# yh-jun/SNR-Aligned_diffSE

Hardware: AMD Instinct MI355X
Metric: utterances/sec (4 s @16 kHz, N=30 PC steps) at 1/2/4/8 MI355X; PESQ delta vs ref (higher is better)
Workload: dtype fp16; 1 GPU; C2: B=32 4 s/16 kHz clips per GPU, N=30 PC steps (reverse_diffusion + ald, 60 NFE/utt), OUVE SDE, NCSN++ nf=128, fp16; global_batch=32, per_gpu_batch=32, seq_len=512, parallelism=dp1 (utterance sharding)

## Files before the change

include/snrse.h:

```cpp
#ifndef SNRSE_H_
#define SNRSE_H_

#include <stddef.h>
#include <stdint.h>

#ifdef __cplusplus
extern "C" {
#endif

typedef struct ihipStream_t* hipStream_t;

enum { SNRSE_F32 = 0, SNRSE_BF16 = 1, SNRSE_F16 = 2, SNRSE_F64 = 3, SNRSE_F32X3 = 4 };

int snrse_abi_version(void);
const char* snrse_build_id(void);
const char* snrse_error_string(int code);
int snrse_device_name(char* buf, int len);

typedef struct snrse_ctx snrse_ctx;
snrse_ctx* snrse_ctx_create(void);
void snrse_ctx_destroy(snrse_ctx* ctx);
int snrse_ctx_set_workspace(snrse_ctx* ctx, void* ptr, size_t bytes);
int snrse_ctx_set_option(snrse_ctx* ctx, const char* name, int value);
int snrse_ctx_get_option(const snrse_ctx* ctx, const char* name, int* value);
int snrse_ctx_probe_begin(snrse_ctx* ctx, int capacity);
int snrse_ctx_probe_read(snrse_ctx* ctx, float* ms, int* kernel, int max, int* n);

int snrse_upfirdn2d(const void* in, void* out, const float* kernel, int major, int in_h, int in_w,
                    int minor, int kh, int kw, int up_x, int up_y, int down_x, int down_y,
                    int pad_x0, int pad_x1, int pad_y0, int pad_y1, int dtype, hipStream_t stream);

int snrse_conv2d(snrse_ctx* ctx, const void* src0, int C0, const void* src1, int C1, int B, int H, int W, int ksize,
                 const void* wgt, const void* sc_src, int Csc, const void* sc_src1, int Csc1,
                 const void* sc_wgt, const float* bias, const float* temb, int temb_stride,
                 const void* res, int res_ld, float out_scale, const float* comb_src,
                 const float* comb_w, const float* comb_b, void* out, int Cout, int out_ld,
                 double* stats, const float* gn_scale, const float* gn_shift, int gn_act, int dtype,
                 int out_f32, hipStream_t stream);

#define SNRSE_STAT_SLOTS 16

int snrse_gn_stats(snrse_ctx* ctx, const void* src0, int C0, const void* src1, int C1, int B, int HW, double* sums,
                   double* sums1, int dtype, hipStream_t stream);

int snrse_gn_scale_shift(const double* sums0, int C0, const double* sums1, int C1, int B, int HW,
                         const float* gamma, const float* beta, int groups, float eps, float* scale,
                         float* shift, hipStream_t stream);

int snrse_gn_apply(const void* src0, int C0, const void* src1, int C1, int B, int H, int W,
                   const double* sums, const double* sums1, const float* gamma, const float* beta,
                   int groups, float eps, int act, int mode, void* out, int dtype, hipStream_t stream);

int snrse_gn_resample(snrse_ctx* ctx, const void* src, int C, int B, int H, int W, const float* scale, const float* shift,
                      int act, int mode, void* out_act, void* out_raw, int dtype, hipStream_t stream);

int snrse_gn_act(const void* src0, int C0, const void* src1, int C1, int B, int HW, const float* scale,
                 const float* shift, int act, void* out, int dtype, hipStream_t stream);

int snrse_set_workspace(void* ptr, size_t bytes);

int snrse_set_option(const char* name, int value);

int snrse_get_option(const char* name, int* value);

int snrse_attention(const void* qkv, void* out, int B, int L, int C, int dtype, hipStream_t stream);

int snrse_temb_mlp(const float* t, const float* Wg, const float* W1, const float* b1, const float* W2,
                   const float* b2, float* temb, int B, int nf, hipStream_t stream);
int snrse_temb_gfp_dense(const float* t, const float* Wg, const float* W1, const float* b1, float* out, int B, int nf,
                         hipStream_t stream);
int snrse_temb_dense(const float* temb, const float* W, const float* bias, float* out, int B, int R, int D,
                     hipStream_t stream);

int snrse_input_conv(snrse_ctx* ctx, const void* x, const void* y, int B, int H, int W, const void* wgt, const float* bias,
                     void* out, float* pyr, double* stats, int dtype, hipStream_t stream);

int snrse_input_conv_x3(snrse_ctx* ctx, const void* x, const void* y, int B, int H, int W, const void* wgt,
                        const float* bias, float* out, float* pyr, double* stats, hipStream_t stream);

int snrse_input_pack(const void* x, const void* y, int B, int H, int W, void* col, float* pyr, int dtype,
                     hipStream_t stream);

int snrse_score_update(const void* pyr, int pyr_f32, const float* out_w, const float* out_b,
                       const float* t, int score_mode, int B, int HW, const void* x, const void* y,
                       const void* noise, uint64_t seed, uint64_t offset, const float* coef,
                       void* x_out, void* xmean_out, void* score_out, hipStream_t stream);

int snrse_sde_update(const void* x, const void* y, const void* score, const void* noise, uint64_t seed,
                     uint64_t offset, const float* coef, int B, int HW, void* x_out, void* xmean_out,
                     hipStream_t stream);

int snrse_axpby_noise(const void* x, const void* y, const void* noise, uint64_t seed, uint64_t offset,
                      const float* coef, int B, int HW, void* out, hipStream_t stream);

int snrse_score_update_rs(const void* pyr, int pyr_f32, const float* out_w, const float* out_b,
                          const float* t, int score_mode, int B, int HW, const void* x, const void* y,
                          const void* noise, const uint64_t* row_seed, uint64_t draw, const float* coef,
                          void* x_out, void* xmean_out, void* score_out, hipStream_t stream);
int snrse_sde_update_rs(const void* x, const void* y, const void* score, const void* noise,
                        const uint64_t* row_seed, uint64_t draw, const float* coef, int B, int HW, void* x_out,
                        void* xmean_out, hipStream_t stream);
int snrse_axpby_noise_rs(const void* x, const void* y, const void* noise, const uint64_t* row_seed,
                         uint64_t draw, const float* coef, int B, int HW, void* out, hipStream_t stream);

int snrse_energy_ratios(const float* s_hat, const float* s, const float* n, int B, int L, double* out,
                        hipStream_t stream);

int snrse_absmax(const float* sig, int B, int L, float* out, hipStream_t stream);

int snrse_energy_ratios_ragged(const float* s_hat, const float* s, const float* n, const int* lengths, int B,
                               int Lstride, double* out, hipStream_t stream);
int snrse_absmax_ragged(const float* sig, const int* lengths, int B, int Lstride, float* out, hipStream_t stream);
int snrse_stft_ragged(const float* sig, const int* lengths, int B, int Lstride, const float* in_div,
                      float in_scale, int Tpad, int mode, void* out, hipStream_t stream);

int snrse_resample_poly(const float* x, const int* lengths, int B, long long stride_in, int up, int down, int half,
                        const float* taps, float* y, long long stride_out, hipStream_t stream);
int snrse_resample_poly_block(void);

int snrse_window_gather(const float* src, const int* lengths, int R, long long stride, const int* table, int nwin,
                        int W, float* out, hipStream_t stream);
int snrse_window_merge(const float* win, int nwin, int W, const int* starts, const unsigned char* silent,
                       const int* first, const int* lengths, int R, const float* fade, int V, float* out,
                       long long stride_out, hipStream_t stream);

int snrse_estoi(const float* x, const float* y, const int* lengths, int B, long long stride, void* work,
                size_t work_bytes, double* out, int* info, hipStream_t stream);
size_t snrse_estoi_workspace(int B, long long stride);
int snrse_estoi_block(void);

int snrse_range_stats(const void* src, int B, long long per, int dtype, float* peak, int* nonfinite,
                      int accumulate, hipStream_t stream);


int snrse_rk45_combine(const double* y, const double* h, const void* const* k, const double* c, int ns, int kdtype,
                       int B, long long n, double* out, float* out32, hipStream_t stream);

int snrse_rk45_rownorm(const void* const* v, const double* c, int ns, int vdtype, const double* m, const double* a,
                       const double* b2, double rtol, double atol, int cplx, int B, long long n, double* partial,
                       double* out, hipStream_t stream);
int snrse_rk45_rownorm_blocks(int B, long long n);

int snrse_rk45_accept(const int* mask, void* y, const void* y_new, long long ywords, void* f, const void* f_new,
                      long long fwords, int B, hipStream_t stream);

int snrse_stft(const float* sig, int B, int L, const float* in_div, float in_scale, int Tpad, int mode,
               void* out, hipStream_t stream);

int snrse_istft(const void* spec, int B, int T, int L, int mode, const float* out_scale, float* frames,
                float* out, hipStream_t stream);

int snrse_spec_transform(const void* in, void* out, long long n, int dir, hipStream_t stream);

int snrse_snrnet(const void* spec, int B, int T, const float* w5, const float* b5, const float* w3,
                 const float* b3, const float* wt1, const float* wt2, const float* wt3, const float* wt4,
                 const float* bt1, const float* bt2, const float* bt3, const float* bt4, const float* wih,
                 const float* bsum, const float* whh, const float* fcw, const float* fcb, float* ws,
                 float* out, hipStream_t stream);
size_t snrse_snrnet_workspace(int B, int T);


int snrse_snr_perturb(const void* x, const void* y, const float* gt, int B, long long per, void* out,
                      hipStream_t stream);
int snrse_snrnet_train_fwd(const void* spec, int B, int T, const float* w5, const float* b5, const float* w3,
                           const float* b3, const float* wt1, const float* wt2, const float* wt3, const float* wt4,
                           const float* bt1, const float* bt2, const float* bt3, const float* bt4, const float* wih,
                           const float* bsum, const float* whh, const float* fcw, const float* fcb, void* tws,
                           float* out, hipStream_t stream);
size_t snrse_snrnet_train_workspace(int B, int T);
int snrse_snrnet_backward(const void* spec, int B, int T, const float* est, const float* dest, const float* w3,
                          const float* wt1, const float* wt2, const float* wt3, const float* wt4, const float* wih,
                          const float* whh, const float* fcw, void* tws, float* dw5, float* db5, float* dw3,
                          float* db3, float* dwt1, float* dwt2, float* dwt3, float* dwt4, float* dbt1, float* dbt2,
                          float* dbt3, float* dbt4, float* dwih, float* dbsum, float* dwhh, float* dfcw, float* dfcb,
                          hipStream_t stream);


int snrse_conv_wgrad(const float* dy, int Cout, const float* x0, int C0, const float* x1, int C1, int B, int H,
                     int W, int ksize, float* dw, hipStream_t stream);
int snrse_conv_wgrad_x3(const float* dy, int Cout, const float* x0, int C0, const float* x1, int C1, int B, int H,
                        int W, int ksize, float* dw, hipStream_t stream);
int snrse_chan_sum(const float* x, int B, int HW, int C, float* out_bc, float* out_c, float scale,
                   hipStream_t stream);
int snrse_gn_moments(const double* st0, int C0, const double* st1, int C1, int B, int HW, int groups, float eps,
                     float* mean, float* rstd, hipStream_t stream);
int snrse_gn_backward(const float* x0, int C0, const float* x1, int C1, const float* dy, int B, int HW,
                      int groups, const float* gamma, const float* beta, const float* mean, const float* rstd,
                      int act, float* R, float* dx0, float* dx1, float* dgamma, float* dbeta, hipStream_t stream);
int snrse_bgemm(const float* A, long long sAb, long long sAm, long long sAk, const float* Bm, long long sBb,
                long long sBk, long long sBn, float* C, long long sCb, long long sCm, long long sCn, const float* bias,
                int batch, int M, int N, int K, float alpha, float beta, hipStream_t stream);
int snrse_softmax_rows(const float* S, float* P, long long rows, int L, float scale, hipStream_t stream);
int snrse_softmax_bwd_rows(const float* P, const float* dP, float* dS, long long rows, int L, float scale,
                           hipStream_t stream);
int snrse_silu(const float* x, float* y, long long n, hipStream_t stream);
int snrse_silu_bwd(const float* x, const float* dy, float* dx, long long n, int accumulate, hipStream_t stream);
int snrse_axpby(const float* x, float* y, long long n, float a, float b, hipStream_t stream);
int snrse_scale_rows(const float* x, const float* s, float* y, int B, long long per, int recip, hipStream_t stream);
int snrse_gfp(const float* t, const float* Wg, int B, int nf, float* out, hipStream_t stream);
int snrse_ct_perturb(const void* x, const void* y, const void* z, const float* wmix, const float* nscale, int B,
                     int HW, int transform, void* mu, void* xt, hipStream_t stream);
int snrse_ct_loss(const void* dnn1, const void* dnn0, const void* x1, const void* x0, const float* coef, int B,
                  int HW, int sqrt_loss, double* loss_b, void* g1, void* g0, hipStream_t stream);
int snrse_adam_ema(const void* tensors, const int* chunk_tensor, const long long* chunk_start, int nchunks,
                   float lr, float beta1, float beta2, float eps, float bias_corr1, float bias_corr2_sqrt,
                   float ema_decay, hipStream_t stream);
int snrse_grad_sumsq(const void* tensors, const int* chunk_tensor, const long long* chunk_start, int nchunks,
                     double* partial, hipStream_t stream);
int snrse_grad_clip_coef(const double* partial, int npartials, float max_norm, float accum_scale, float* out,
                         hipStream_t stream);
int snrse_adam_ema_scaled(const void* tensors, const int* chunk_tensor, const long long* chunk_start, int nchunks,
                          float lr, float beta1, float beta2, float eps, float bias_corr1, float bias_corr2_sqrt,
                          float ema_decay, const float* gscale, hipStream_t stream);
int snrse_grad_pack(const void* tensors, const int* chunk_tensor, const long long* chunk_start, int nchunks,
                    const long long* flat_off, float scale, float* flat, hipStream_t stream);


int snrse_active_window_sums(const float* c, const float* n, const int* lengths, int B, long long stride, int W,
                             double* wsums, double* partials, float* nmax, hipStream_t stream);
int snrse_active_windows_per_block(void);
int snrse_active_finalize(const double* wsums, const double* partials, const float* nmax, const int* lengths, int B,
                          long long stride, int W, const double* snr_db, double* out, hipStream_t stream);
int snrse_snr_mix(const float* c, const float* n, const int* lengths, int B, long long stride, const double* gain,
                  int gain_stride, float* n_out, float* y_out, float* ymax, hipStream_t stream);
int snrse_scale_to_pcm16(const float* c, const float* n1, const float* y, const int* lengths, int B, long long stride,
                         const float* ymax, float* c_f, float* n_f, float* y_f, short* c_q, short* n_q, short* y_q,
                         double* scale, hipStream_t stream);

#ifdef __cplusplus
}
#endif
#endif
```

snr-aligned_diffse_amd/csrc/abi.cpp:

```cpp
#include <hip/hip_runtime.h>

#include <new>

#include "common.h"

extern "C" int snrse_abi_version(void) { return 2; }

#ifndef SNRSE_BUILD_ID
#define SNRSE_BUILD_ID "unknown"
#endif
extern "C" const char* snrse_build_id(void) { return SNRSE_BUILD_ID; }

extern "C" const char* snrse_error_string(int code) { return hipGetErrorString((hipError_t)code); }

extern "C" int snrse_device_name(char* buf, int len) {
  int dev = 0;
  hipError_t e = hipGetDevice(&dev);
  if (e != hipSuccess) return (int)e;
  hipDeviceProp_t prop;
  e = hipGetDeviceProperties(&prop, dev);
  if (e != hipSuccess) return (int)e;
  int i = 0;
  for (const char* s = prop.gcnArchName; *s && i < len - 1; ++s) buf[i++] = *s;
  if (len > 0) buf[i] = 0;
  return 0;
}

namespace {
snrse_ctx g_default_ctx;

bool name_is(const char* a, const char* b) {
  int i = 0;
  while (a[i] && a[i] == b[i]) ++i;
  return a[i] == 0 && b[i] == 0;
}

int* option_field(snrse_ctx& c, const char* name) {
  if (name_is(name, "conv_variant")) return &c.conv_variant;
  if (name_is(name, "splitk")) return &c.splitk;
  if (name_is(name, "splitk_target")) return &c.splitk_target;
  if (name_is(name, "epi_nt")) return &c.epi_nt;
  if (name_is(name, "epi_nt_mb")) return &c.epi_nt_mb;
  if (name_is(name, "h5_specialise")) return &c.h5_specialise;
  if (name_is(name, "h5_tw")) return &c.h5_tw;
  if (name_is(name, "stats_zeroed")) return &c.stats_zeroed;
  if (name_is(name, "resample_variant")) return &c.resample_variant;
  if (name_is(name, "resample_nt")) return &c.resample_nt;
  if (name_is(name, "resample_down_rows")) return &c.resample_down_rows;
  if (name_is(name, "x3_tile")) return &c.x3_tile;
  if (name_is(name, "x3_spread")) return &c.x3_spread;
  if (name_is(name, "ic_lds")) return &c.ic_lds;
  if (name_is(name, "x3_nt")) return &c.x3_nt;
  if (name_is(name, "x3_tw")) return &c.x3_tw;
  if (name_is(name, "head_small")) return &c.head_small;
  if (name_is(name, "head_part")) return &c.head_part;
  if (name_is(name, "gn_slice")) return &c.gn_slice;
  return nullptr;
}

int set_option(snrse_ctx& c, const char* name, int value) {
  if (!name) return SNRSE_EINVAL;
  int* f = option_field(c, name);
  if (!f) return SNRSE_EINVAL;
  if (name_is(name, "splitk_target") || name_is(name, "epi_nt_mb")) value = value > 0 ? value : 256;
  if (name_is(name, "stats_zeroed")) value = value ? 1 : 0;
  *f = value;
  return 0;
}

int get_option(const snrse_ctx& c, const char* name, int* value) {
  if (!name || !value) return SNRSE_EINVAL;
  if (const int* f = option_field(const_cast<snrse_ctx&>(c), name)) { *value = *f; return 0; }
  if (name_is(name, "halo_kernel")) { *value = 5; return 0; }
  if (name_is(name, "last_kernel")) { *value = c.last_kernel; return 0; }
  if (name_is(name, "last_ksplit")) { *value = c.last_ksplit; return 0; }
  if (name_is(name, "last_epi_nt")) { *value = c.last_epi_nt; return 0; }
  if (name_is(name, "last_chunks")) { *value = c.last_chunks; return 0; }
  if (name_is(name, "last_tw")) { *value = c.last_tw; return 0; }
  return SNRSE_EINVAL;
}

int set_workspace(snrse_ctx& c, void* ptr, size_t bytes) {
  if (!ptr && bytes) return SNRSE_EINVAL;
  c.ws = (float*)ptr;
  c.ws_bytes = ptr ? bytes : 0;
  return 0;
}
}

__attribute__((visibility("hidden"))) snrse_ctx* snrse_ctx_resolve(snrse_ctx* c) { return c ? c : &g_default_ctx; }

namespace {
void probe_free(snrse_ctx& c) {
  for (int i = 0; i < 2 * c.probe_cap; ++i) (void)hipEventDestroy(c.probe_ev[i]);
  delete[] c.probe_ev;
  delete[] c.probe_kernel;
  c.probe_ev = nullptr;
  c.probe_kernel = nullptr;
  c.probe_cap = c.probe_n = 0;
}
}

__attribute__((visibility("hidden"))) int snrse_ctx_probe_mark(snrse_ctx& c, hipStream_t s, bool end) {
  if (c.probe_n >= c.probe_cap) return 0;
  if (end) {
    c.probe_kernel[c.probe_n] = c.last_kernel;
    return (int)hipEventRecord(c.probe_ev[2 * c.probe_n++ + 1], s);
  }
  return (int)hipEventRecord(c.probe_ev[2 * c.probe_n], s);
}

extern "C" int snrse_ctx_probe_begin(snrse_ctx* ctx, int capacity) {
  snrse_ctx& c = *snrse_ctx_resolve(ctx);
  probe_free(c);
  if (capacity <= 0) return 0;
  c.probe_ev = new (std::nothrow) hipEvent_t[2 * (size_t)capacity];
  c.probe_kernel = new (std::nothrow) int[capacity];
  if (!c.probe_ev || !c.probe_kernel) {
    delete[] c.probe_ev;
    delete[] c.probe_kernel;
    c.probe_ev = nullptr;
    c.probe_kernel = nullptr;
    return (int)hipErrorOutOfMemory;
  }
  for (int i = 0; i < 2 * capacity; ++i) {
    const hipError_t e = hipEventCreateWithFlags(&c.probe_ev[i], hipEventDisableSystemFence);
    if (e != hipSuccess) {
      c.probe_cap = i / 2;
      for (int j = 2 * c.probe_cap; j < i; ++j) (void)hipEventDestroy(c.probe_ev[j]);
      probe_free(c);
      return (int)e;
    }
  }
  c.probe_cap = capacity;
  c.probe_n = 0;
  return 0;
}

extern "C" int snrse_ctx_probe_read(snrse_ctx* ctx, float* ms, int* kernel, int max, int* n) {
  snrse_ctx& c = *snrse_ctx_resolve(ctx);
  if (!n) return SNRSE_EINVAL;
  const int m = c.probe_n < max ? c.probe_n : max;
  for (int i = 0; i < m; ++i) {
    hipError_t e = hipEventSynchronize(c.probe_ev[2 * i + 1]);
    if (e != hipSuccess) return (int)e;
    if (ms) {
      e = hipEventElapsedTime(&ms[i], c.probe_ev[2 * i], c.probe_ev[2 * i + 1]);
      if (e != hipSuccess) return (int)e;
    }
    if (kernel) kernel[i] = c.probe_kernel[i];
  }
  *n = m;
  return 0;
}

extern "C" snrse_ctx* snrse_ctx_create(void) {
  snrse_ctx* c = new (std::nothrow) snrse_ctx(g_default_ctx);
  if (!c) return nullptr;
  c->ws = nullptr;
  c->ws_bytes = 0;
  c->last_kernel = 0;
  c->last_ksplit = 1;
  c->last_epi_nt = 0;
  c->last_chunks = 1;
  c->last_tw = 0;
  c->probe_ev = nullptr;
  c->probe_kernel = nullptr;
  c->probe_cap = c->probe_n = 0;
  return c;
}

extern "C" void snrse_ctx_destroy(snrse_ctx* ctx) {
  if (ctx) probe_free(*ctx);
  delete ctx;
}

extern "C" int snrse_ctx_set_workspace(snrse_ctx* ctx, void* ptr, size_t bytes) {
  return set_workspace(*snrse_ctx_resolve(ctx), ptr, bytes);
}
extern "C" int snrse_ctx_set_option(snrse_ctx* ctx, const char* name, int value) {
  return set_option(*snrse_ctx_resolve(ctx), name, value);
}
extern "C" int snrse_ctx_get_option(const snrse_ctx* ctx, const char* name, int* value) {
  return get_option(*snrse_ctx_resolve(const_cast<snrse_ctx*>(ctx)), name, value);
}

extern "C" int snrse_set_workspace(void* ptr, size_t bytes) { return set_workspace(g_default_ctx, ptr, bytes); }
extern "C" int snrse_set_option(const char* name, int value) { return set_option(g_default_ctx, name, value); }
extern "C" int snrse_get_option(const char* name, int* value) { return get_option(g_default_ctx, name, value); }
```

snr-aligned_diffse_amd/csrc/common.h:

```cpp
#pragma once
#include <hip/hip_runtime.h>
#include <stdint.h>

#define SNRSE_DEV __device__ __forceinline__

typedef uint16_t bf16_t;

typedef __attribute__((ext_vector_type(8))) __bf16 bf16x8_mfma;
typedef __attribute__((ext_vector_type(4))) float f32x4;
typedef __attribute__((ext_vector_type(4))) unsigned int u32x4;

SNRSE_DEV float bf2f(bf16_t v) { return __uint_as_float(((uint32_t)v) << 16); }

SNRSE_DEV bf16_t f2bf(float f) {
  uint32_t u = __float_as_uint(f);
  if ((u & 0x7f800000u) == 0x7f800000u && (u & 0x007fffffu)) return (bf16_t)((u >> 16) | 0x40);
  u += 0x7fffu + ((u >> 16) & 1u);
  return (bf16_t)(u >> 16);
}

SNRSE_DEV uint32_t pack_bf16x2(float lo, float hi) {
  typedef __attribute__((ext_vector_type(2))) __bf16 bf16x2_t;
  const bf16x2_t v = {(__bf16)lo, (__bf16)hi};
  return __builtin_bit_cast(uint32_t, v);
}

struct f16_t {
  uint16_t bits;
};
typedef __attribute__((ext_vector_type(8))) _Float16 f16x8_mfma;
typedef __attribute__((ext_vector_type(2))) _Float16 f16x2_t;

template <typename T> struct H16;
template <> struct H16<bf16_t> {
  SNRSE_DEV static float lo(uint32_t v) { return __uint_as_float(v << 16); }
  SNRSE_DEV static float hi(uint32_t v) { return __uint_as_float(v & 0xffff0000u); }
  SNRSE_DEV static uint32_t pack(float a, float b) { return pack_bf16x2(a, b); }
  SNRSE_DEV static f32x4 mfma(const u32x4& a, const u32x4& b, f32x4 acc) {
    return __builtin_amdgcn_mfma_f32_16x16x32_bf16(__builtin_bit_cast(bf16x8_mfma, a),
                                                   __builtin_bit_cast(bf16x8_mfma, b), acc, 0, 0, 0);
  }
};
template <> struct H16<f16_t> {
  SNRSE_DEV static float lo(uint32_t v) { return (float)__builtin_bit_cast(f16x2_t, v)[0]; }
  SNRSE_DEV static float hi(uint32_t v) { return (float)__builtin_bit_cast(f16x2_t, v)[1]; }
  SNRSE_DEV static uint32_t pack(float a, float b) {
    const f16x2_t v = {(_Float16)a, (_Float16)b};
    return __builtin_bit_cast(uint32_t, v);
  }
  SNRSE_DEV static f32x4 mfma(const u32x4& a, const u32x4& b, f32x4 acc) {
    return __builtin_amdgcn_mfma_f32_16x16x32_f16(__builtin_bit_cast(f16x8_mfma, a),
                                                  __builtin_bit_cast(f16x8_mfma, b), acc, 0, 0, 0);
  }
};
template <typename T>
SNRSE_DEV void unpack8(const u32x4& r, float* v) {
#pragma unroll
  for (int i = 0; i < 4; ++i) {
    v[2 * i] = H16<T>::lo(r[i]);
    v[2 * i + 1] = H16<T>::hi(r[i]);
  }
}
template <typename T>
SNRSE_DEV u32x4 pack8(const float* v) {
  u32x4 r;
#pragma unroll
  for (int i = 0; i < 4; ++i) r[i] = H16<T>::pack(v[2 * i], v[2 * i + 1]);
  return r;
}

template <typename T> struct Elem;
template <> struct Elem<float> {
  static constexpr int kBytes = 4;
  SNRSE_DEV static float to_f(float v) { return v; }
  SNRSE_DEV static float from_f(float v) { return v; }
};
template <> struct Elem<bf16_t> {
  static constexpr int kBytes = 2;
  SNRSE_DEV static float to_f(bf16_t v) { return bf2f(v); }
  SNRSE_DEV static bf16_t from_f(float v) { return f2bf(v); }
};
template <> struct Elem<f16_t> {
  static constexpr int kBytes = 2;
  SNRSE_DEV static float to_f(f16_t v) { return (float)__builtin_bit_cast(_Float16, v.bits); }
  SNRSE_DEV static f16_t from_f(float v) { return f16_t{__builtin_bit_cast(uint16_t, (_Float16)v)}; }
};

SNRSE_DEV float silu(float x) { return x * __builtin_amdgcn_rcpf(1.0f + __expf(-x)); }
constexpr float kNegLog2e = -1.44269504088896341f;
constexpr float kNegInvLn2 = -1.44269504088896341f;
SNRSE_DEV float silu_z(float z) {
  return z * __builtin_amdgcn_rcpf(fmaf(__builtin_amdgcn_exp2f(z), kNegInvLn2, kNegInvLn2));
}

SNRSE_DEV float silu_exact(float x) { return x / (1.0f + expf(-x)); }

SNRSE_DEV float wave_sum(float v) {
#pragma unroll
  for (int o = 32; o > 0; o >>= 1) v += __shfl_xor(v, o, 64);
  return v;
}
SNRSE_DEV float wave_max(float v) {
#pragma unroll
  for (int o = 32; o > 0; o >>= 1) v = fmaxf(v, __shfl_xor(v, o, 64));
  return v;
}
template <int N>
SNRSE_DEV float bfly_sum(float (&p)[N], int lane) {
  static_assert(N >= 1 && N <= 64 && (N & (N - 1)) == 0, "N: power of two <= 64");
  int lb = 0;
#pragma unroll
  for (int n = N; n > 1; n >>= 1, ++lb) {
    const bool hi = (lane >> lb) & 1;
#pragma unroll
    for (int i = 0; i < n / 2; ++i) {
      const float keep = hi ? p[2 * i + 1] : p[2 * i];
      const float send = hi ? p[2 * i] : p[2 * i + 1];
      p[i] = keep + __shfl_xor(send, 1 << lb, 64);
    }
  }
  float v = p[0];
#pragma unroll
  for (int b = lb; b < 6; ++b) v += __shfl_xor(v, 1 << b, 64);
  return v;
}

SNRSE_DEV int xcd_block_id(int bid, int nblocks) {
  const int q8 = nblocks >> 3, r8 = nblocks & 7, xcd = bid & 7, pos = bid >> 3;
  return (xcd < r8 ? xcd * (q8 + 1) : r8 * (q8 + 1) + (xcd - r8) * q8) + pos;
}

SNRSE_DEV float dot4(const f32x4& a, const f32x4& b) {
  return fmaf(a[0], b[0], fmaf(a[1], b[1], fmaf(a[2], b[2], a[3] * b[3])));
}

SNRSE_DEV double wave_sum_d(double v) {
#pragma unroll
  for (int o = 32; o > 0; o >>= 1) v += __shfl_xor(v, o, 64);
  return v;
}

enum { SNRSE_F32 = 0, SNRSE_BF16 = 1, SNRSE_F16 = 2, SNRSE_F64 = 3, SNRSE_F32X3 = 4 };
inline bool snrse_is16(int dtype) { return dtype == SNRSE_BF16 || dtype == SNRSE_F16; }

#define SNRSE_STAT_SLOTS 16

struct snrse_ctx {
  int conv_variant = 0;
  int splitk = 1;
  int splitk_target = 256;
  int epi_nt = 2;
  int epi_nt_mb = 256;
  int h5_specialise = 1;
  int h5_tw = 0;
  int stats_zeroed = 0;
  int resample_variant = 0;
  int resample_nt = 0;
  int resample_down_rows = 4;
  int x3_tile = 0;
  int x3_tw = 0;
  int x3_nt = 1;
  int x3_spread = 2;
  int head_small = 1;
  int head_part = 1;
  int gn_slice = 1;
  int ic_lds = 3;
  float* ws = nullptr;
  size_t ws_bytes = 0;
  int last_kernel = 0, last_ksplit = 1, last_epi_nt = 0, last_chunks = 1, last_tw = 0;
  hipEvent_t* probe_ev = nullptr;
  int* probe_kernel = nullptr;
  int probe_cap = 0, probe_n = 0;
};
int snrse_ctx_probe_mark(snrse_ctx& c, hipStream_t s, bool end);
snrse_ctx* snrse_ctx_resolve(snrse_ctx* c);
SNRSE_DEV size_t stat_idx(int b, int slot, int c, int C) {
  return (((size_t)b * SNRSE_STAT_SLOTS + slot) * C + c) * 2;
}
SNRSE_DEV void stat_fold(const double* st, int b, int c, int C, double& s, double& ss) {
#pragma unroll 4
  for (int k = 0; k < SNRSE_STAT_SLOTS; ++k) {
    const double* q = st + stat_idx(b, k, c, C);
    s += q[0];
    ss += q[1];
  }
}

#define SNRSE_RET(expr)                              \
  do {                                               \
    hipError_t _e = (expr);                          \
    if (_e != hipSuccess) return (int)_e;            \
  } while (0)
#define SNRSE_LAUNCH_CHECK() SNRSE_RET(hipGetLastError())
#define SNRSE_EINVAL ((int)hipErrorInvalidValue)
```

snr-aligned_diffse_amd/csrc/conv.hip:

```cpp
#include "conv_common.h"

#include <algorithm>
#include <type_traits>

using namespace snrse_conv;

namespace {

template <int NWM, int BN>
SNRSE_DEV void block_stats_flush(const ConvParams& p, const float* red, int blk_b, int blk_n0) {
  asm volatile("s_waitcnt lgkmcnt(0)" ::: "memory");
  __builtin_amdgcn_s_barrier();
  const int slot = blockIdx.x & (SNRSE_STAT_SLOTS - 1);
  for (int t = threadIdx.x; t < 2 * BN; t += blockDim.x) {
    float a = 0.f;
#pragma unroll
    for (int w = 0; w < NWM; ++w) a += red[w * 2 * BN + t];
    if (blk_n0 + (t >> 1) < p.Cout)
      unsafeAtomicAdd(&p.stats[stat_idx(blk_b, slot, blk_n0 + (t >> 1), p.Cout) + (t & 1)], (double)a);
  }
}

template <typename TO, int NWM, int BN, bool DEFER = false, int LA = 8>
SNRSE_DEV void epilogue_lds(const ConvParams& p, const f32x4 (&acc)[4][4], int mb, int nb, int lane, float* stage,
// ... 894 lines not shown
        wait_vm(infl ? HOPS : 0);
        __builtin_amdgcn_s_barrier();
        char* const nxt = ring + (SLOT2 - so);
        if constexpr (k < 8) {
          wtap(c0 + (2 * k + 2) / 9, (2 * k + 2) % 9, nxt);
          wtap(c0 + (2 * k + 3) / 9, (2 * k + 3) % 9, nxt + TAPB);
        } else {
          if (more) {
            wtap(c0 + 2, 0, nxt);
            wtap(c0 + 2, 1, nxt + TAPB);
          } else if (cbs > 0) {
            wtap(cbm, 4, nxt);
          }
        }
        infl = false;
        if constexpr (k == 0) {
          halo_load(c1);
          infl = true;
        }
        if constexpr (k == 4) {
          if (pf1) {
            halo_load(c1 + 1);
            infl = true;
          }
        }
        const char* const sl_ = ring + so;
        auto piece_after = [&](int d, int t) {
          const int c = c0 + d;
          if (t < 4 || t > 7) return;
          if (d == 1 && !pf1) return;
          char* const nb_ = smem + ((c + 1) & 1) * HBYTES;
          const bool tr = c + 1 < cbm;
          if (t == 4) { halo_piece(nb_, 0, tr); halo_piece(nb_, 1, tr); }
          if (t == 5) { halo_piece(nb_, 2, tr); halo_piece(nb_, 3, tr); }
          if (t == 6) halo_piece(nb_, 4, tr);
          if (t == 7) halo_piece(nb_, 5, tr);
        };
        tap_mfma(smem + ((c0 + da) & 1) * HBYTES, sl_, ta);
        piece_after(da, ta);
        __builtin_amdgcn_sched_barrier(0);
        tap_mfma(smem + ((c0 + db) & 1) * HBYTES, sl_ + TAPB, tb);
        piece_after(db, tb);
        __builtin_amdgcn_sched_barrier(0);
        so = SLOT2 - so;
      });
    }
    for (int c = cbm; c < ncb; ++c) {
      asm volatile("s_waitcnt vmcnt(0) lgkmcnt(0)" ::: "memory");
      __builtin_amdgcn_s_barrier();
      if (c + 1 < ncb) wtap(c + 1, 4, ring + (SLOT2 - so));
      if (c + 1 < ncb) halo_load(c + 1);
      tap_mfma(smem + (c & 1) * HBYTES, ring + so, 4);
      if (c + 1 < ncb) {
        asm volatile("s_waitcnt vmcnt(0)" ::: "memory");
        char* const nb_ = smem + ((c + 1) & 1) * HBYTES;
#pragma unroll
        for (int j = 0; j < HJ; ++j) halo_piece(nb_, j, false);
      }
      so = SLOT2 - so;
    }
  } else if constexpr (SPR == 1) {
    int q = 0;
    for (int c = 0; c < cbm; ++c) {
      const bool tr = c + 1 < cbm;
      char* const nb_ = smem + ((c + 1) & 1) * HBYTES;
      const char* const hb = smem + (c & 1) * HBYTES;
#pragma unroll
      for (int tp = 0; tp < 9; ++tp, ++q) {
        if (tp == 1) asm volatile("s_waitcnt vmcnt(%0)" ::"n"(2 + HOPS) : "memory");
        else asm volatile("s_waitcnt vmcnt(2)" ::: "memory");
        asm volatile("s_waitcnt lgkmcnt(0)" ::: "memory");
        __builtin_amdgcn_s_barrier();
        wload(q + 2);
        if (tp == 0) halo_load(c + 1 < ncb ? c + 1 : c);
        tap_mfma(hb, ring + (q % 3) * TAPB, tp);
        if (tp >= 2 && tp - 2 < HJ) halo_piece(nb_, tp - 2, tr);
      }
    }
    for (int c = cbm; c < ncb; ++c, ++q) {
      const int qa = q - 2, qb = q - 1;
      const bool fa = qa >= 0 && (qa >= 9 * cbm || qa % 9 == 0), fb = qb >= 0 && (qb >= 9 * cbm || qb % 9 == 0);
      x3h_vm_wait(2 + HOPS * (int)fa + HOPS * (int)fb);
      asm volatile("s_waitcnt lgkmcnt(0)" ::: "memory");
      __builtin_amdgcn_s_barrier();
      wload(q + 2);
      halo_load(c + 1 < ncb ? c + 1 : c);
      tap_mfma(smem + (c & 1) * HBYTES, ring + (q % 3) * TAPB, 4);
      asm volatile("s_waitcnt vmcnt(0)" ::: "memory");
      char* const nb_ = smem + ((c + 1) & 1) * HBYTES;
#pragma unroll
      for (int j = 0; j < HJ; ++j) halo_piece(nb_, j, false);
    }
  } else
  for (int q = 0; q < nq; ++q) {
    const int c = phase_chunk(q), tp = phase_tap(q);
    x3h_vm_wait(HOPS * (int)first_with_next(q - 2) + 2 * (int)(q + 1 < nq) + HOPS * (int)first_with_next(q - 1));
    asm volatile("s_waitcnt lgkmcnt(0)" ::: "memory");
    __builtin_amdgcn_s_barrier();
    if (q + 2 < nq) wload(q + 2);
    const bool pre = first_with_next(q);
    if (pre) halo_load(c + 1);
    const char* hb = smem + (c & 1) * HBYTES;
    const char* sb = ring + (q % 3) * TAPB;
    const int dy = tp / 3 - 1, dx = tp - (tp / 3) * 3 - 1;
    const int hbase = (wr * RW + dy + 1) * HC + dx + 1 + lrow;
    u32x4 ah[4], al[4], bh[4], bl[4];
#pragma unroll
    for (int i = 0; i < 4; ++i) {
      const int hr = hbase + (16 * i / TW) * HC + (16 * i) % TW;
      ah[i] = *(const u32x4*)(hb + swz(hr, lg));
      al[i] = *(const u32x4*)(hb + swz(hr, 4 + lg));
    }
#pragma unroll
    for (int j = 0; j < 4; ++j) {
      bh[j] = *(const u32x4*)(sb + swz(wc * 64 + j * 16 + lrow, lg));
      bl[j] = *(const u32x4*)(sb + swz(wc * 64 + j * 16 + lrow, 4 + lg));
    }
#pragma unroll
    for (int i = 0; i < 4; ++i)
#pragma unroll
      for (int j = 0; j < 4; ++j) {
        acc[i][j] = mfma_chunk<bf16_t>(ah[i], bh[j], acc[i][j]);
        acc[i][j] = mfma_chunk<bf16_t>(ah[i], bl[j], acc[i][j]);
        acc[i][j] = mfma_chunk<bf16_t>(al[i], bh[j], acc[i][j]);
      }
    const int q0 = q < 9 * cbm ? q - tp : q;
    const bool last_of_chunk = c < cbm ? tp == 8 : true;
    const bool store_now = c + 1 < ncb && (c < cbm ? tp == 1 : true);
    if (store_now) {
      x3h_vm_wait(q == q0 ? 0 : 2 * (int)(q0 + 3 < nq));
      halo_store(c + 1);
    }
    (void)last_of_chunk;
  }
  asm volatile("s_waitcnt vmcnt(0) lgkmcnt(0)" ::: "memory");
  __builtin_amdgcn_s_barrier();
  const int mb = (bb * p.H + h0 + wr * RW) * p.W + w0;
  if constexpr (TW == 64)
    epilogue_lds<float, 4, 128>(p, acc, mb, n0 + wc * 64, lane, (float*)(smem + wid * (64 * 68 * 4)),
                                (float*)(smem + 8 * (64 * 68 * 4)), wr, bb, n0, min(TW, p.W - w0));
  else
    epilogue_img<float, 4, 128, false, EF, TW>(p, acc, mb, n0 + wc * 64, lane, (float*)(smem + wid * (64 * 68 * 4)),
                                                 (float*)(smem + 8 * (64 * 68 * 4)), wr, bb, n0, p.W - TW);
}

template <int BM, int BN, typename T, typename TO>
__global__ __launch_bounds__(512) void conv_glds_kernel(ConvParams p) {
  constexpr int WM = BM / 64, WN = BN / 64;
  static_assert(WM * WN == 8, "8 waves");
  constexpr int FM = 4, FN = 4, TM = 64, TN = 64;
  constexpr int STAGES = 3;
  constexpr int A_BYTES = BM * 128, B_BYTES = BN * 128, STAGE = A_BYTES + B_BYTES;
  constexpr int AJ = BM / 64, BJ = BN / 64;
  constexpr int KT = 64;
  extern __shared__ __attribute__((aligned(16))) char smem[];

  const int tid = threadIdx.x, lane = tid & 63;
  const int wid = __builtin_amdgcn_readfirstlane(tid >> 6);
  const int wm = wid / WN, wn = wid % WN;
  const int wg = xcd_block_id(blockIdx.x, gridDim.x);
  const int ks = wg % p.ksplit, tl = wg / p.ksplit;
  const int m0 = (tl / p.ntn) * BM;
  const int n0 = (tl % p.ntn) * BN;

  const int HW = p.H * p.W;
  const int Cin = p.C0 + p.C1;
  const int cblocks = Cin / KT;
  const int nk0 = p.ksize * p.ksize * cblocks;
  const int Csc_all = p.Csc + p.Csc1;
  const int nk = nk0 + (p.sc_src ? Csc_all / KT : 0);
  const int K1 = p.ksize * p.ksize * Cin;
  const int half = p.ksize >> 1;
  const int slot = lane & 7;

  int a_pix[AJ], a_h[AJ], a_w[AJ], a_ch[AJ];
  bool a_ok[AJ];
#pragma unroll
  for (int j = 0; j < AJ; ++j) {
    const int row = (wid * AJ + j) * 8 + (lane >> 3);
    const int m = m0 + row;
    a_ok[j] = m < p.M;
    const int mm = a_ok[j] ? m : 0;
    const int b = mm / HW, rem = mm - b * HW;
    a_h[j] = rem / p.W;
    a_w[j] = rem - a_h[j] * p.W;
    a_pix[j] = mm;
    a_ch[j] = slot ^ (row & 7);
  }

#define SNRSE_ISSUE(KT_, STAGE_)                                                                      \
  do {                                                                                              \
    const int kt_ = (KT_);                                                                          \
    char* sa_ = smem + (STAGE_) * STAGE;                                                            \
    char* sb_ = sa_ + A_BYTES;                                                                      \
    int cs_, cc_, dy_, dx_, wld_, koff_;                                                            \
    const void* abase_;                                                                             \
    long long abytes_;                                                                              \
    const void* wbase_;                                                                             \
    long long wbytes_;                                                                              \
    if (kt_ < nk0) {                                                                                \
      const int tap_ = kt_ / cblocks;                                                               \
      const int c_ = (kt_ - tap_ * cblocks) * KT;                                                   \
      dy_ = tap_ / p.ksize - half;                                                                  \
      dx_ = tap_ - (tap_ / p.ksize) * p.ksize - half;                                               \
      const bool u1_ = c_ >= p.C0;                                                                  \
      abase_ = u1_ ? p.src1 : p.src0;                                                               \
      abytes_ = u1_ ? p.bytes1 : p.bytes0;                                                          \
      cs_ = u1_ ? p.C1 : p.C0;                                                                      \
      cc_ = u1_ ? c_ - p.C0 : c_;                                                                   \
      wbase_ = p.wgt;                                                                               \
      wbytes_ = p.wbytes;                                                                           \
      wld_ = K1;                                                                                    \
      koff_ = tap_ * Cin + c_;                                                                      \
    } else {                                                                                        \
      const int c_ = (kt_ - nk0) * KT;                                                              \
      const bool u1_ = c_ >= p.Csc;                                                                 \
      abase_ = u1_ ? p.sc_src1 : p.sc_src;                                                          \
      abytes_ = u1_ ? p.sc_bytes1 : p.sc_bytes0;                                                    \
      cs_ = u1_ ? p.Csc1 : p.Csc;                                                                   \
      cc_ = u1_ ? c_ - p.Csc : c_;                                                                  \
      dy_ = 0;                                                                                      \
      dx_ = 0;                                                                                      \
      wbase_ = p.sc_wgt;                                                                            \
      wbytes_ = p.sc_wbytes;                                                                        \
      wld_ = Csc_all;                                                                               \
      koff_ = c_;                                                                                   \
    }                                                                                               \
    const __amdgpu_buffer_rsrc_t ra_ = make_rsrc(abase_, abytes_);                                  \
    const __amdgpu_buffer_rsrc_t rb_ = make_rsrc(wbase_, wbytes_);                                  \
    const int shift_ = dy_ * p.W + dx_;                                                             \
    _Pragma("unroll") for (int j = 0; j < AJ; ++j) {                                                \
      const int hh_ = a_h[j] + dy_, ww_ = a_w[j] + dx_;                                             \
      const bool ok_ = a_ok[j] && hh_ >= 0 && hh_ < p.H && ww_ >= 0 && ww_ < p.W;                   \
      const unsigned voff_ =                                                                        \
          ok_ ? (unsigned)(((a_pix[j] + shift_) * cs_ + cc_ + a_ch[j] * 8) * 2) : 0x80000000u;      \
      __builtin_amdgcn_raw_ptr_buffer_load_lds(                                                     \
          ra_, (__attribute__((address_space(3))) void*)(sa_ + (wid * AJ + j) * 1024), 16, voff_, 0, 0, 0); \
    }                                                                                               \
    _Pragma("unroll") for (int j = 0; j < BJ; ++j) {                                                \
      const int row_ = (wid * BJ + j) * 8 + (lane >> 3);                                            \
      const int chk_ = slot ^ (row_ & 7);                                                           \
      const unsigned voff_ = (unsigned)(((n0 + row_) * wld_ + koff_ + chk_ * 8) * 2);               \
      __builtin_amdgcn_raw_ptr_buffer_load_lds(                                                     \
          rb_, (__attribute__((address_space(3))) void*)(sb_ + (wid * BJ + j) * 1024), 16, voff_, 0, 0, 0); \
    }                                                                                               \
  } while (0)

  f32x4 acc[FM][FN];
#pragma unroll
  for (int i = 0; i < FM; ++i)
#pragma unroll
    for (int j = 0; j < FN; ++j) acc[i][j] = f32x4{0.f, 0.f, 0.f, 0.f};

  const int kb = (int)((long long)ks * nk / p.ksplit), ke = (int)((long long)(ks + 1) * nk / p.ksplit);
  SNRSE_ISSUE(kb, 0);
  if (ke - kb > 1) SNRSE_ISSUE(kb + 1, 1);
  const int lrow = lane & 15, lg = lane >> 4;
  int stage = 0;
  for (int kt = kb; kt < ke; ++kt) {
    if (kt + 1 < ke)
      asm volatile("s_waitcnt vmcnt(%0)" ::"n"(AJ + BJ) : "memory");
    else
      asm volatile("s_waitcnt vmcnt(0)" ::: "memory");
    __builtin_amdgcn_s_barrier();
    if (kt + 2 < ke) SNRSE_ISSUE(kt + 2, stage == 0 ? 2 : stage - 1);
    const char* sa = smem + stage * STAGE;
    const char* sb = sa + A_BYTES;
#pragma unroll
    for (int s = 0; s < 2; ++s) {
      u32x4 af[FM], bfr[FN];
#pragma unroll
      for (int i = 0; i < FM; ++i) af[i] = *(const u32x4*)(sa + swz(wm * TM + i * 16 + lrow, 4 * s + lg));
#pragma unroll
      for (int j = 0; j < FN; ++j) bfr[j] = *(const u32x4*)(sb + swz(wn * TN + j * 16 + lrow, 4 * s + lg));
#pragma unroll
      for (int i = 0; i < FM; ++i)
#pragma unroll
        for (int j = 0; j < FN; ++j) acc[i][j] = mfma_chunk<T>(af[i], bfr[j], acc[i][j]);
    }
    stage = stage == STAGES - 1 ? 0 : stage + 1;
  }
#undef SNRSE_ISSUE
  if (p.ksplit > 1) {
    float* const wsp = p.ws + (size_t)ks * p.M * p.Cout;
#pragma unroll
    for (int i = 0; i < FM; ++i)
#pragma unroll
      for (int e = 0; e < 4; ++e) {
        const int m = m0 + wm * TM + i * 16 + lg * 4 + e;
        if (m < p.M) {
#pragma unroll
          for (int j = 0; j < FN; ++j) wsp[(size_t)m * p.Cout + n0 + wn * TN + j * 16 + lrow] = acc[i][j][e];
        }
      }
    return;
  }
  asm volatile("s_waitcnt vmcnt(0) lgkmcnt(0)" ::: "memory");
  __builtin_amdgcn_s_barrier();
  const int b_lo = m0 / HW, b_hi = (min(m0 + BM, p.M) - 1) / HW;
  epilogue_lds<TO, WM, BN, false, sizeof(TO) == 2 ? 8 : 1>(p, acc, m0 + wm * TM, n0 + wn * TN, lane, (float*)(smem + wid * (64 * 68 * 4)),
                           (float*)(smem + 8 * (64 * 68 * 4)), wm, b_lo == b_hi ? b_lo : -1, n0);
}

template <typename TO>
__global__ __launch_bounds__(256) void conv_splitk_finalize(ConvParams p, int ppb) {
  __shared__ float red[16 * 256];
  const int HW = p.H * p.W;
  const int nbi = (HW + ppb - 1) / ppb;
  const int b = blockIdx.x / nbi;
  const int px0 = (blockIdx.x - b * nbi) * ppb, px1 = min(HW, px0 + ppb);
  const int cl = (threadIdx.x & 15) * 8, r0 = threadIdx.x >> 4;
  const int n = blockIdx.y * 128 + cl;
  float add[8], cw[8][4], cb[8], s1[8], s2[8];
#pragma unroll
  for (int k = 0; k < 8; ++k) {
    add[k] = (p.bias ? p.bias[n + k] : 0.f) + (p.temb ? p.temb[(size_t)b * p.temb_stride + n + k] : 0.f);
    s1[k] = 0.f;
    s2[k] = 0.f;
    cb[k] = 0.f;
    cw[k][0] = cw[k][1] = cw[k][2] = cw[k][3] = 0.f;
    if (p.comb_src) {
      cw[k][0] = p.comb_w[(n + k) * 4 + 0];
      cw[k][1] = p.comb_w[(n + k) * 4 + 1];
      cw[k][2] = p.comb_w[(n + k) * 4 + 2];
      cw[k][3] = p.comb_w[(n + k) * 4 + 3];
      cb[k] = p.comb_b[n + k];
    }
  }
  const size_t plane = (size_t)p.M * p.Cout;
  for (int px = px0 + r0; px < px1; px += 16) {
    const size_t m = (size_t)b * HW + px;
    const float* w = p.ws + m * p.Cout + n;
    f32x4 a0 = *(const f32x4*)w, a1 = *(const f32x4*)(w + 4);
    int s = 1;
    for (; s + 4 <= p.ksplit; s += 4) {
      f32x4 q[4][2];
#pragma unroll
      for (int u = 0; u < 4; ++u) {
        q[u][0] = *(const f32x4*)(w + (s + u) * plane);
        q[u][1] = *(const f32x4*)(w + (s + u) * plane + 4);
      }
#pragma unroll
      for (int u = 0; u < 4; ++u) {
        a0 += q[u][0];
        a1 += q[u][1];
      }
    }
    for (; s < p.ksplit; ++s) {
      a0 += *(const f32x4*)(w + s * plane);
      a1 += *(const f32x4*)(w + s * plane + 4);
    }
    float v[8];
#pragma unroll
    for (int k = 0; k < 4; ++k) {
      v[k] = a0[k] + add[k];
      v[4 + k] = a1[k] + add[4 + k];
    }
    if (p.res) {
      if constexpr (sizeof(TO) == 2) {
        epi_residual<TO>(*(const u32x4*)((const TO*)p.res + m * p.res_ld + n), v);
      } else {
        const float* rp = (const float*)p.res + m * p.res_ld + n;
#pragma unroll
        for (int k = 0; k < 8; ++k) v[k] += rp[k];
      }
    }
#pragma unroll
    for (int k = 0; k < 8; ++k) v[k] *= p.out_scale;
    if (p.comb_src) {
      const f32x4 q = *(const f32x4*)(p.comb_src + m * 4);
#pragma unroll
      for (int k = 0; k < 8; ++k) v[k] += q[0] * cw[k][0] + q[1] * cw[k][1] + q[2] * cw[k][2] + q[3] * cw[k][3] + cb[k];
    }
    if constexpr (sizeof(TO) == 2) {
      *(u32x4*)((TO*)p.out + m * p.out_ld + n) = epi_pack<TO>(v);
    } else {
      float* op = (float*)p.out + m * p.out_ld + n;
#pragma unroll
      for (int k = 0; k < 8; ++k) op[k] = v[k];
    }
#pragma unroll
    for (int k = 0; k < 8; ++k) {
      s1[k] += v[k];
      s2[k] = fmaf(v[k], v[k], s2[k]);
    }
  }
  if (p.stats) {
#pragma unroll
    for (int k = 0; k < 8; ++k) {
      red[r0 * 256 + (cl + k) * 2] = s1[k];
      red[r0 * 256 + (cl + k) * 2 + 1] = s2[k];
    }
    __syncthreads();
    const int t = threadIdx.x;
    float a = 0.f;
#pragma unroll
    for (int r = 0; r < 16; ++r) a += red[r * 256 + t];
    unsafeAtomicAdd(&p.stats[stat_idx(b, blockIdx.x & (SNRSE_STAT_SLOTS - 1), blockIdx.y * 128 + (t >> 1), p.Cout) +
                             (t & 1)],
                    (double)a);
  }
}


template <typename T, typename TO, int GNM, int EF, int TW, bool SCD>
__global__ __launch_bounds__(256, 2) void conv_halo5_kernel(ConvParams p) {
  constexpr int TH = 256 / TW, HC = TW + 2;
  constexpr int RW = TH / 4;
  constexpr int HROWS = (TH + 2) * HC;
  constexpr int HJ = (HROWS + 63) / 64;
  constexpr int HALO_BYTES = HROWS * 64;
  constexpr int TAPB = 128 * 64;
  constexpr int SLOT = 3 * TAPB;
  constexpr int KT = 32;
  static_assert(64 * HJ >= HROWS, "halo rows");
  extern __shared__ __attribute__((aligned(16))) char smem[];
  char* const halo = smem;
  char* const ring = smem + HALO_BYTES;
  float* const gnl = (float*)(smem + HALO_BYTES + 2 * SLOT + 1024);
  constexpr bool REGEPI = sizeof(TO) == 2;
  constexpr int MAIN_BYTES = HALO_BYTES + 2 * SLOT + 1280;
  constexpr int STAGE_BYTES = 4 * (64 * 68 * 4);

  const int tid = threadIdx.x, lane = tid & 63;
  const int wid = __builtin_amdgcn_readfirstlane(tid >> 6);
#ifdef SNRSE_STAMPS
  constexpr int kStampOff = REGEPI ? MAIN_BYTES + 4096
                                   : (MAIN_BYTES > STAGE_BYTES + 4096 ? MAIN_BYTES : STAGE_BYTES + 4096);
  unsigned long long* const lst = (unsigned long long*)(smem + kStampOff) + wid * 32;
#endif
  SNRSE_STAMP(0);
  const int wg = xcd_block_id(blockIdx.x, gridDim.x);
  const int n0 = (wg % p.ntn) * 128;
  int tile = wg / p.ntn;
  const int ntw = p.W / TW, nth = p.H / TH;
  const int w0 = (tile % ntw) * TW;
  tile /= ntw;
  const int h0 = (tile % nth) * TH;
  const int bb = tile / nth;

  const int Cin = p.C0 + p.C1;
  const int cbm = Cin / KT;
  const int Csc_all = p.Csc + p.Csc1;
  const int cbs = p.sc_src ? Csc_all / KT : 0;
  const int nq = 3 * cbm + cbs;
  const int K1 = 9 * Cin;
  const int hcol = tid & 3;

  const int rl = lane >> 2, swz8 = ((lane & 3) ^ ((rl >> 1) & 3)) * 8;
  const __amdgpu_buffer_rsrc_t wrsrc = make_rsrc(p.wgt, p.wbytes);
  const int wr0 = REGEPI ? 8 * rl + wid : wid * 16 + rl;
  constexpr int WODD = REGEPI ? 4 : 64;
  const unsigned wlane = (unsigned)(((n0 + wr0) * K1 + swz8) * 2);
  const unsigned wrow64 = (unsigned)(WODD * K1 * 2), wtap = (unsigned)(Cin * 2);
  using lds_ptr = __attribute__((address_space(3))) void*;
  auto dma_w = [&](auto k_, unsigned vl, unsigned soff, char* dst) {
    constexpr int k = decltype(k_)::value;
    __builtin_amdgcn_raw_ptr_buffer_load_lds(wrsrc, (lds_ptr)(dst + (k >> 1) * TAPB + (wid + 4 * (k & 1)) * 1024), 16,
                                             vl, soff + (k & 1) * wrow64 + (k >> 1) * wtap, 0, 0);
  };
  auto woff = [&](int c, int g) { return (unsigned)((3 * g * Cin + c * KT) * 2); };

  u32x4 hv[HJ];
  f32x4 gnv;
  auto gn_load = [&](int c) {
    if constexpr (GNM > 0) {
      if (tid < 16)
        gnv = *(const f32x4*)((tid < 8 ? p.gn_scale : p.gn_shift) + (size_t)bb * Cin + c * KT + (tid & 7) * 4);
    }
  };

  static_for<6>([&](auto k) { dma_w(k, wlane, 0u, ring); });
  gn_load(0);
  __builtin_amdgcn_sched_barrier(0);

  int hpix[HJ];
  bool hok[HJ];
#pragma unroll
  for (int j = 0; j < HJ; ++j) {
    const int hr = (tid >> 2) + 64 * j;
    const int hy = hr / HC, hx = hr - (hr / HC) * HC;
    const int ih = h0 + hy - 1, iw = w0 + hx - 1;
    hok[j] = hr < HROWS && ih >= 0 && ih < p.H && iw >= 0 && iw < p.W;
    hpix[j] = (bb * p.H + ih) * p.W + iw;
  }

#define SNRSE_HALO5_LOADS(BASE_, BYTES_, CS_, CC_)                                                     \
  do {                                                                                              \
    const __amdgpu_buffer_rsrc_t r_ = make_rsrc((BASE_), (BYTES_));                                 \
    const int cs_ = (CS_), cc_ = (CC_) + hcol * 8;                                                  \
    _Pragma("unroll") for (int j = 0; j < HJ; ++j) {                                                \
      const int voff_ = hok[j] ? (hpix[j] * cs_ + cc_) * 2 : (int)0x80000000;                       \
      hv[j] = __builtin_amdgcn_raw_buffer_load_b128(r_, voff_, 0, 0);                               \
    }                                                                                               \
  } while (0)
  auto halo_load = [&](int c) {
    const int ch = c * KT;
    const bool s1 = ch >= p.C0;
    SNRSE_HALO5_LOADS(s1 ? p.src1 : p.src0, s1 ? p.bytes1 : p.bytes0, s1 ? p.C1 : p.C0, s1 ? ch - p.C0 : ch);
  };
#undef SNRSE_HALO5_LOADS
  auto gn_publish = [&]() {
    if constexpr (GNM > 0) {
      if (tid < 16) {
        f32x4 g = gnv;
        if constexpr (GNM == 2) g *= kNegLog2e;
        *(f32x4*)(gnl + tid * 4) = g;
      }
    }
  };
  auto halo_store = [&](int c) {
    const bool tr = GNM > 0;
    float gsc[8], gsh[8];
    if constexpr (GNM > 0) {
      if (tr) {
        const f32x4 s0 = *(const f32x4*)(gnl + hcol * 8), s1 = *(const f32x4*)(gnl + hcol * 8 + 4);
        const f32x4 t0 = *(const f32x4*)(gnl + 32 + hcol * 8), t1 = *(const f32x4*)(gnl + 32 + hcol * 8 + 4);
#pragma unroll
        for (int i = 0; i < 4; ++i) { gsc[i] = s0[i]; gsc[4 + i] = s1[i]; gsh[i] = t0[i]; gsh[4 + i] = t1[i]; }
      }
    }
#pragma unroll
    for (int j = 0; j < HJ; ++j) {
      const int hr = (tid >> 2) + 64 * j;
      if (j == HJ - 1 && hr >= HROWS) break;
      u32x4 v = hv[j];
      if constexpr (GNM > 0) {
        if (tr) v = gn_xform8<T, GNM>(v, gsc, gsh, hok[j]);
      }
      *(u32x4*)(halo + swz64(hr, hcol)) = v;
    }
  };
  f32x4 acc[2][4][4];
#pragma unroll
  for (int h = 0; h < 2; ++h)
#pragma unroll
    for (int i = 0; i < 4; ++i)
#pragma unroll
      for (int j = 0; j < 4; ++j) acc[h][i][j] = f32x4{0.f, 0.f, 0.f, 0.f};
  const int lrow = lane & 15, lg = lane >> 4;
  auto vm_after_dma = [&]() { __builtin_amdgcn_s_waitcnt(0x0f76); };


  if constexpr (SCD) {
    const int kq = cbs / cbm, kr = cbs - kq * cbm;
    int krem = 0;
    auto nsc_next = [&]() {
      krem += kr;
      const bool wrap = krem >= cbm;
      if (wrap) krem -= cbm;
      return kq + (wrap ? 1 : 0);
    };
    auto kind_of = [](int s, int k, int& su) -> int {
      su = 0;
      if (k >= 3) {
        if (s == 0 || s == 2 || s == 4) return s >> 1;
        su = s <= 3 ? s >> 1 : s - 3;
        return 3;
      }
      if (s < 2) return s;
      if (k == 0) return 2;
      if (k == 1) {
        if (s == 2) return 2;
        return 3;
      }
      if (s == 3) return 2;
      su = s == 2 ? 0 : 1;
      return 3;
    };
    auto m2_pos = [](int k) { return k >= 3 ? 4 : k == 2 ? 3 : 2; };
    const __amdgpu_buffer_rsrc_t scrsrc = make_rsrc(p.sc_wgt, p.sc_wbytes);
    const __amdgpu_buffer_rsrc_t xrsrc0 = make_rsrc(p.sc_src, p.sc_bytes0), xrsrc1 = make_rsrc(p.sc_src1, p.sc_bytes1);
    const unsigned sclane = (unsigned)(((n0 + wr0) * Csc_all + swz8) * 2);
    const unsigned scrow64 = (unsigned)(WODD * Csc_all * 2);
    const int trow = wid * 16 + rl;
    const int xpix = (bb * p.H + h0 + trow / TW) * p.W + w0 + trow % TW;
    halo_load(0);
    if constexpr (GNM > 0) {
      gn_publish();
      __syncthreads();
    }
    halo_store(0);
    const bool w0g = GNM > 0 && wid == 0;
    bool halo_inflight = false;
    int c = 0, pos = 0, k = nsc_next(), ub = 0;
    int su, kind = kind_of(0, k, su);
    for (int q = 0; q < nq; ++q) {
      int c2 = c, pos2 = pos + 1, k2 = k, ub2 = ub;
      if (pos2 == 3 + k) { c2 = c + 1; pos2 = 0; ub2 = ub + k; k2 = c2 < cbm ? nsc_next() : 0; }
      int su2;
      const int kind2 = kind_of(pos2, k2, su2);
      if (halo_inflight) {
        if (w0g) asm volatile("s_waitcnt vmcnt(%0) lgkmcnt(0)" ::"n"(HJ + 1) : "memory");
        else asm volatile("s_waitcnt vmcnt(%0) lgkmcnt(0)" ::"n"(HJ) : "memory");
      } else {
        asm volatile("s_waitcnt vmcnt(0) lgkmcnt(0)" ::: "memory");
      }
      __builtin_amdgcn_s_barrier();
      char* const nx = ring + ((q + 1) & 1) * SLOT;
      __amdgpu_buffer_rsrc_t Rc, Rn;
      unsigned Vc, Vn, Sc, Sn, Oc, On, DPn;
      int DDn;
      char* Dc = nx + wid * 1024;
      char* Dn = Dc + TAPB;
      if (kind2 < 3) {
        const bool fin = q + 1 >= nq;
        Rc = Rn = wrsrc;
        Vc = Vn = fin ? wlane | 0x80000000u : wlane;
        Sc = fin ? 0u : woff(c2, kind2);
        Sn = Sc + wtap; DPn = wtap; DDn = TAPB;
        Oc = On = wrow64;
      } else {
        const int kb = (ub2 + su2) * KT;
        const bool one = kb >= p.Csc;
        const int cs = one ? p.Csc1 : p.Csc, cb = one ? kb - p.Csc : kb;
        const unsigned xstep = (unsigned)((64 / TW) * p.W * cs * 2);
        Rc = scrsrc; Vc = sclane; Sc = (unsigned)(kb * 2); Oc = scrow64;
        Rn = one ? xrsrc1 : xrsrc0;
        Vn = (unsigned)((xpix * cs + swz8) * 2);
        Sn = (unsigned)(cb * 2); On = xstep; DPn = 2 * xstep; DDn = 8192;
      }
      auto dma_pair = [&]() {
        __builtin_amdgcn_raw_ptr_buffer_load_lds(Rc, (lds_ptr)Dc, 16, Vc, Sc, 0, 0);
        __builtin_amdgcn_raw_ptr_buffer_load_lds(Rc, (lds_ptr)(Dc + 4096), 16, Vc, Sc + Oc, 0, 0);
        Rc = Rn; Vc = Vn; Sc = Sn; Oc = On; Dc = Dn;
        Sn += DPn; Dn += DDn;
      };
      const char* sl = ring + (q & 1) * SLOT;
      const bool mainph = kind < 3;
      const char* abuf = mainph ? halo : sl + TAPB;
      const int ntap = mainph ? 3 : 1, rs = mainph ? HC : TW;
      const int arow0 = mainph ? (wid * RW + kind) * HC + lrow : wid * RW * TW + lrow;
      auto tap_body = [&](int jt, auto gap_) {
        constexpr bool gap = decltype(gap_)::value;
        const int arow = arow0 + jt;
        const char* sb = sl + jt * TAPB;
        u32x4 af[4], bfr[8];
#pragma unroll
        for (int i = 0; i < 4; ++i) af[i] = *(const u32x4*)(abuf + swz64(arow + (16 * i / TW) * rs + (16 * i) % TW, lg));
#pragma unroll
        for (int j = 0; j < 8; ++j) bfr[j] = *(const u32x4*)(sb + swz64(j * 16 + lrow, lg));
        static_for<32>([&](auto m_) {
          constexpr int m = decltype(m_)::value, h = m >> 4, i = (m >> 2) & 3, j = m & 3;
          acc[h][i][j] = mfma_chunk<T>(af[i], bfr[h * 4 + j], acc[h][i][j]);
          if constexpr (gap && (m & 7) == 7 && m < 24) dma_pair();
        });
        if constexpr (gap) {
#pragma unroll
          for (int u = 0; u < 3; ++u) {
            __builtin_amdgcn_sched_group_barrier(0x008, 8, 0);
            __builtin_amdgcn_sched_group_barrier(0x020, 2, 0);
          }
          __builtin_amdgcn_sched_group_barrier(0x008, 8, 0);
        }
      };
      tap_body(0, std::true_type{});
#pragma nounroll
      for (int jt = 1; jt < ntap; ++jt) tap_body(jt, std::false_type{});
      if (kind == 0 && c + 1 < cbm) {
        vm_after_dma();
        halo_load(c + 1);
        gn_load(c + 1);
        halo_inflight = true;
      } else {
        halo_inflight = false;
      }
      if (c + 1 < cbm) {
        if (kind == 2) {
          gn_publish();
          if (k == 0) {
            asm volatile("s_waitcnt lgkmcnt(0)" ::: "memory");
            __builtin_amdgcn_s_barrier();
            vm_after_dma();
            halo_store(c + 1);
          }
        } else if (kind == 3 && pos == m2_pos(k) + 1) {
          vm_after_dma();
          halo_store(c + 1);
        }
      }
      c = c2; pos = pos2; k = k2; ub = ub2; kind = kind2; su = su2;
    }
  } else {
  halo_load(0);
  if constexpr (GNM > 0) {
    gn_publish();
    __syncthreads();
  }
  halo_store(0);
  SNRSE_STAMP(1);
  bool halo_inflight = false;
  const bool w0g = GNM > 0 && wid == 0;
  int c = 0, g = 0;
  unsigned soff = woff(0, 1);
  const unsigned soff_g = 3 * wtap, soff_c = (unsigned)(2 * KT) - 6 * wtap;
  for (int q = 0; q < nq; ++q) {
    const bool first = g == 0, last = g == 2;
    if (halo_inflight) {
      if (w0g) asm volatile("s_waitcnt vmcnt(%0) lgkmcnt(0)" ::"n"(HJ + 1) : "memory");
      else asm volatile("s_waitcnt vmcnt(%0) lgkmcnt(0)" ::"n"(HJ) : "memory");
    } else {
      asm volatile("s_waitcnt vmcnt(0) lgkmcnt(0)" ::: "memory");
    }
    __builtin_amdgcn_s_barrier();
    SNRSE_STAMP(2 + 2 * (q & 15));
    const bool fin = q + 1 >= nq;
    const unsigned vl = fin ? wlane | 0x80000000u : wlane, so = fin ? 0u : soff;
    char* const nx = ring + ((q + 1) & 1) * SLOT;
    const char* sl = ring + (q & 1) * SLOT;
    const int hrow = (wid * RW + g) * HC + lrow;
    static_for<3>([&](auto jt_) {
      constexpr int jt = decltype(jt_)::value;
      const int hbase = hrow + jt;
      const char* sb = sl + jt * TAPB;
      u32x4 af[4], bfr[8];
#pragma unroll
      for (int i = 0; i < 4; ++i) af[i] = *(const u32x4*)(halo + swz64(hbase + (16 * i / TW) * HC + (16 * i) % TW, lg));
#pragma unroll
      for (int j = 0; j < 8; ++j) bfr[j] = *(const u32x4*)(sb + swz64(j * 16 + lrow, lg));
      static_for<32>([&](auto m_) {
        constexpr int m = decltype(m_)::value, h = m >> 4, i = (m >> 2) & 3, j = m & 3;
        acc[h][i][j] = mfma_chunk<T>(af[i], bfr[h * 4 + j], acc[h][i][j]);
        if constexpr (jt < 2 && (m & 7) == 7 && m < 24)
          dma_w(std::integral_constant<int, 3 * jt + (m >> 3)>{}, vl, so, nx);
      });
    });
    static_assert(sizeof(T) == 2, "one MFMA per mfma_chunk");
#pragma unroll
    for (int t = 0; t < 2; ++t) {
#pragma unroll
      for (int u = 0; u < 3; ++u) {
        __builtin_amdgcn_sched_group_barrier(0x008, 8, 0);
        __builtin_amdgcn_sched_group_barrier(0x020, 1, 0);
      }
      __builtin_amdgcn_sched_group_barrier(0x008, 8, 0);
    }
    __builtin_amdgcn_sched_group_barrier(0x008, 32, 0);
    SNRSE_STAMP(3 + 2 * (q & 15));
    if (first && c + 1 < cbm) {
      vm_after_dma();
      halo_load(c + 1);
      gn_load(c + 1);
      halo_inflight = true;
    } else {
      halo_inflight = false;
    }
    if (last && c + 1 < cbm) {
      gn_publish();
      asm volatile("s_waitcnt lgkmcnt(0)" ::: "memory");
      __builtin_amdgcn_s_barrier();
      vm_after_dma();
      halo_store(c + 1);
    }
    soff += g == 1 ? soff_c : soff_g;
    if (last) { g = 0; ++c; }
    else ++g;
  }
  }
  SNRSE_STAMP(28);
#ifdef SNRSE_H5_SKIP_EPI
  if (p.M > 0) {
    asm volatile("s_waitcnt vmcnt(0)" ::: "memory");
    return;
  }
#endif
  const int mrow = (bb * p.H + h0 + wid * RW) * p.W + w0;
  if constexpr (REGEPI) {
    float* const red = (float*)(smem + MAIN_BYTES);
    epilogue_reg<TO, EF, TW>(p, acc, mrow, n0, lane, red + wid * 256, bb, p.W - TW);
    SNRSE_STAMP(26);
    SNRSE_STAMP(27);
    if (EF < 0 ? p.stats != nullptr : (EF & EF_STATS) != 0) block_stats_flush<4, 128>(p, red, bb, n0);
  } else {
    float add0[16 / sizeof(TO)], add1[16 / sizeof(TO)];
    epi_add<TO, EF>(p, n0, lane, bb, add0);
    epi_add<TO, EF>(p, n0 + 64, lane, bb, add1);
    asm volatile("s_waitcnt vmcnt(0) lgkmcnt(0)" ::: "memory");
    __builtin_amdgcn_s_barrier();
    float* const stage = (float*)(smem + wid * (64 * 68 * 4));
    float* const red = (float*)(smem + STAGE_BYTES);
    epilogue_img<TO, 4, 128, true, EF, TW, 2>(p, acc[0], mrow, n0, lane, stage, red, wid, bb, n0, p.W - TW, add0);
    asm volatile("s_waitcnt lgkmcnt(0)" ::: "memory");
    __builtin_amdgcn_wave_barrier();
    SNRSE_STAMP(26);
    epilogue_img<TO, 4, 128, true, EF, TW, 2>(p, acc[1], mrow, n0 + 64, lane, stage, red, wid, bb, n0, p.W - TW, add1);
    SNRSE_STAMP(27);
    if (EF < 0 ? p.stats != nullptr : (EF & EF_STATS) != 0) block_stats_flush<4, 128>(p, red, bb, n0);
  }
#ifdef SNRSE_STAMPS
  {
    unsigned long long st_[29];
    if (lane == 0)
      for (int i = 0; i < 29; ++i) st_[i] = lst[i];
    unsigned long long t_end;
    asm volatile("s_waitcnt vmcnt(0)\n\ts_memtime %0\n\ts_waitcnt lgkmcnt(0)" : "=s"(t_end)::"memory");
    unsigned hw, xcc;
    asm volatile("s_getreg_b32 %0, hwreg(HW_REG_HW_ID)" : "=s"(hw));
    asm volatile("s_getreg_b32 %0, hwreg(HW_REG_XCC_ID)" : "=s"(xcc));
    if (lane == 0 && p.stamps) {
      unsigned long long* g = p.stamps + ((size_t)blockIdx.x * 8 + wid) * 32;
      for (int i = 0; i < 29; ++i) g[i] = st_[i];
      g[29] = t_end;
      g[30] = hw;
      g[31] = xcc;
    }
  }
#endif
}


template <auto K, typename... Args>
int launch_dyn_lds(dim3 grid, dim3 block, size_t lds, hipStream_t s, const Args&... args) {
  static const hipError_t attr = hipFuncSetAttribute((const void*)K, hipFuncAttributeMaxDynamicSharedMemorySize, (int)lds);
  SNRSE_RET(attr);
  hipLaunchKernelGGL(K, grid, block, lds, s, args...);
  return (int)hipGetLastError();
}

template <typename TO>
int launch_splitk_finalize(const ConvParams& p, hipStream_t s) {
  const int HW = p.H * p.W, ppb = 64;
  hipLaunchKernelGGL((conv_splitk_finalize<TO>), dim3(p.B * ((HW + ppb - 1) / ppb), p.Cout / 128), dim3(256), 0, s, p,
                     ppb);
  return (int)hipGetLastError();
}

inline int k_tiles(const ConvParams& p, int KT) {
  return p.ksize * p.ksize * ((p.C0 + p.C1) / KT) + (p.sc_src ? (p.Csc + p.Csc1) / KT : 0);
}

inline int stream_output(const snrse_ctx& cx, long long bytes) {
  return cx.epi_nt == 2 ? bytes > ((long long)cx.epi_nt_mb << 20) : cx.epi_nt;
}

template <typename T, typename TO, int GNM, int EF, int TW, bool SCD>
int launch_halo5_ef(ConvParams p, int grid, hipStream_t s) {
  constexpr size_t main_lds = (256 / TW + 2) * (TW + 2) * 64 + 2 * 3 * 128 * 64 + 1024 + 256;
  constexpr size_t epi_lds = 4 * (64 * 68 * 4) + 4 * 128 * 2 * 4;
  constexpr size_t used_lds = sizeof(TO) == 2 ? main_lds + 4 * 128 * 2 * 4 : (main_lds > epi_lds ? main_lds : epi_lds);
#ifdef SNRSE_STAMPS
  constexpr size_t lds = used_lds + 1024;
#else
  constexpr size_t lds = used_lds;
#endif
  static_assert(lds <= 80 * 1024, "two workgroups per CU");
  return launch_dyn_lds<conv_halo5_kernel<T, TO, GNM, EF, TW, SCD>>(dim3(grid), dim3(256), lds, s, p);
}

template <typename T, typename TO, int GNM, int TW>
int launch_halo5_gn(ConvParams p, hipStream_t s, snrse_ctx& cx) {
  p.ntn = p.Cout / 128;
  p.epi_nt = stream_output(cx, (long long)p.M * p.out_ld * (long long)sizeof(TO));
  cx.last_epi_nt = p.epi_nt;
  const int tiles = p.B * (p.H / (256 / TW)) * (p.W / TW) * p.ntn;
  const int grid = tiles;
  const bool scd = p.sc_src != nullptr;
  if constexpr (sizeof(TO) == 2 && GNM != 1) {
    if (cx.h5_specialise && p.bias) {
#define SNRSE_H5_EF(F) \
  case (F): return launch_halo5_ef<T, TO, GNM, (F), TW, false>(p, grid, s);
#define SNRSE_H5_EFS(F) \
  case (F): return launch_halo5_ef<T, TO, GNM, (F), TW, true>(p, grid, s);
      if (!scd) {
        switch (epi_flags(p)) {
          SNRSE_H5_EF(EF_TEMB | EF_STATS)
          SNRSE_H5_EF(EF_TEMB | EF_STATS | EF_NT)
          SNRSE_H5_EF(EF_RES | EF_STATS)
          SNRSE_H5_EF(EF_RES | EF_STATS | EF_NT)
          SNRSE_H5_EF(EF_STATS)
          SNRSE_H5_EF(EF_STATS | EF_NT)
          SNRSE_H5_EF(EF_TEMB)
          default: break;
        }
      } else {
        switch (epi_flags(p)) {
          SNRSE_H5_EFS(EF_STATS)
          SNRSE_H5_EFS(EF_STATS | EF_NT)
          SNRSE_H5_EFS(EF_COMB | EF_STATS)
          default: break;
        }
      }
#undef SNRSE_H5_EF
#undef SNRSE_H5_EFS
    }
  }
  return scd ? launch_halo5_ef<T, TO, GNM, EF_RT, TW, true>(p, grid, s)
             : launch_halo5_ef<T, TO, GNM, EF_RT, TW, false>(p, grid, s);
}

template <typename T, typename TO, int TW>
int launch_halo5_tw(ConvParams p, hipStream_t s, snrse_ctx& cx) {
  cx.last_tw = TW;
  if (!p.gn_scale) return launch_halo5_gn<T, TO, 0, TW>(p, s, cx);
  if (!p.gn_act) return launch_halo5_gn<T, TO, 1, TW>(p, s, cx);
  return launch_halo5_gn<T, TO, 2, TW>(p, s, cx);
}

inline bool halo_tile32(const ConvParams& p) { return p.H % 8 == 0 && p.W % 32 == 0; }
inline bool halo_tile64(const ConvParams& p) { return p.H % 4 == 0 && p.W % 64 == 0; }

template <typename T, typename TO>
int launch_halo5(ConvParams p, hipStream_t s, snrse_ctx& cx) {
  if (halo_tile32(p) && cx.h5_tw != 64) return launch_halo5_tw<T, TO, 32>(p, s, cx);
  return launch_halo5_tw<T, TO, 64>(p, s, cx);
}

int choose_ksplit(const ConvParams& p, int tiles, int nk, const snrse_ctx& cx, int min_kt = 4) {
  if (!cx.splitk || !cx.ws || tiles >= cx.splitk_target * 3 / 4) return 1;
  int s = (cx.splitk_target + tiles - 1) / tiles;
  if (s > nk / min_kt) s = nk / min_kt;
  const size_t plane = (size_t)p.M * p.Cout * sizeof(float);
  if ((size_t)s * plane > cx.ws_bytes) s = (int)(cx.ws_bytes / plane);
  return s >= 2 ? s : 1;
}

template <typename T, typename TO, int BM, int BN, int WM, int WN>
int launch_conv(ConvParams p, int npad, hipStream_t s, snrse_ctx& cx) {
  p.ntn = npad / BN;
  const int tiles = ((p.M + BM - 1) / BM) * p.ntn;
  p.ksplit = (sizeof(T) == 4 && BN == 128 && p.Cout % 128 == 0)
                 ? choose_ksplit(p, tiles, k_tiles(p, ConvTraits<T>::KT), cx, 2) : 1;
  p.ws = cx.ws;
  cx.last_ksplit = p.ksplit;
  const size_t lds = (size_t)2 * (BM + BN) * 128;
  hipLaunchKernelGGL((conv_mfma_kernel<T, TO, BM, BN, WM, WN>), dim3(tiles * p.ksplit), dim3(64 * WM * WN), lds, s, p);
  if (p.ksplit == 1) return (int)hipGetLastError();
  SNRSE_LAUNCH_CHECK();
  return launch_splitk_finalize<TO>(p, s);
}

template <int BM, int BN, int WM, int WN>
int launch_x3(ConvParams p, hipStream_t s, snrse_ctx& cx) {
  constexpr size_t main_lds = (size_t)2 * (BM + BN) * 128;
  constexpr size_t epi_lds = (BM / WM == 64 && BN / WN == 64) ? (size_t)WM * WN * 64 * 68 * 4 + WM * BN * 2 * 4 : 0;
  constexpr size_t lds = main_lds > epi_lds ? main_lds : epi_lds;
  p.ntn = (p.Cout + BN - 1) / BN;
  const int tiles = ((p.M + BM - 1) / BM) * p.ntn;
  p.ksplit = BN == 128 ? choose_ksplit(p, tiles, k_tiles(p, SplitBf16Opnd::KT), cx, 2) : 1;
  p.ws = cx.ws;
  cx.last_ksplit = p.ksplit;
  const int rc = launch_dyn_lds<conv_x3_kernel<BM, BN, WM, WN>>(dim3(tiles * p.ksplit), dim3(64 * WM * WN), lds, s, p);
  if (rc || p.ksplit == 1) return rc;
  return launch_splitk_finalize<float>(p, s);
}

template <int GNM, int SPR, int TWV, int EF = EF_RT>
int launch_x3h_ef(ConvParams p, hipStream_t s, int tiles) {
  p.ntn = p.Cout / 128;
  p.ksplit = 1;
  return launch_dyn_lds<conv_x3h_kernel<GNM, SPR, TWV, EF>>(dim3(tiles), dim3(512), X3G<TWV, SPR>::LDS, s, p);
}

template <int GNM, int SPR, int TWV>
int launch_x3h_gn(const ConvParams& p, hipStream_t s, int tiles, bool spec) {
  if constexpr (GNM != 1 && SPR == 2 && TWV == 32) {
    if (spec && p.bias) {
      switch (epi_flags(p)) {
        case EF_TEMB | EF_STATS: return launch_x3h_ef<GNM, SPR, TWV, EF_TEMB | EF_STATS>(p, s, tiles);
        case EF_TEMB | EF_STATS | EF_NT: return launch_x3h_ef<GNM, SPR, TWV, EF_TEMB | EF_STATS | EF_NT>(p, s, tiles);
        case EF_RES | EF_STATS: return launch_x3h_ef<GNM, SPR, TWV, EF_RES | EF_STATS>(p, s, tiles);
        case EF_RES | EF_STATS | EF_NT: return launch_x3h_ef<GNM, SPR, TWV, EF_RES | EF_STATS | EF_NT>(p, s, tiles);
        case EF_STATS: return launch_x3h_ef<GNM, SPR, TWV, EF_STATS>(p, s, tiles);
        case EF_STATS | EF_NT: return launch_x3h_ef<GNM, SPR, TWV, EF_STATS | EF_NT>(p, s, tiles);
        case EF_COMB | EF_STATS: return launch_x3h_ef<GNM, SPR, TWV, EF_COMB | EF_STATS>(p, s, tiles);
        case EF_COMB | EF_STATS | EF_NT: return launch_x3h_ef<GNM, SPR, TWV, EF_COMB | EF_STATS | EF_NT>(p, s, tiles);
        default: break;
      }
    }
  }
  return launch_x3h_ef<GNM, SPR, TWV>(p, s, tiles);
}

template <int SPR, int TWV>
int launch_x3h_spr(const ConvParams& p, hipStream_t s, int tiles, bool spec) {
  if (!p.gn_scale) return launch_x3h_gn<0, SPR, TWV>(p, s, tiles, spec);
  if (!p.gn_act) return launch_x3h_gn<1, SPR, TWV>(p, s, tiles, spec);
  return launch_x3h_gn<2, SPR, TWV>(p, s, tiles, spec);
}

int launch_x3h(const ConvParams& p, hipStream_t s, int tiles, int spread, int tw, bool spec) {
  if (spread == 2 && !(tw == 32 && ((p.C0 + p.C1) / 32) % 2 == 0)) spread = 1;
  if (tw == 32) {
    if (spread == 2) return launch_x3h_spr<2, 32>(p, s, tiles, spec);
    return spread ? launch_x3h_spr<1, 32>(p, s, tiles, spec) : launch_x3h_spr<0, 32>(p, s, tiles, spec);
  }
  return spread ? launch_x3h_spr<1, 64>(p, s, tiles, spec) : launch_x3h_spr<0, 64>(p, s, tiles, spec);
}

template <int BM, int BN, typename T, typename TO>
int launch_glds(ConvParams p, hipStream_t s, snrse_ctx& cx) {
  constexpr size_t lds = (size_t)3 * (BM + BN) * 128;
  p.ntn = p.Cout / BN;
  const int ntm = (p.M + BM - 1) / BM;
  p.ksplit = choose_ksplit(p, ntm * p.ntn, k_tiles(p, 64), cx);
  p.ws = cx.ws;
  cx.last_ksplit = p.ksplit;
  const int rc = launch_dyn_lds<conv_glds_kernel<BM, BN, T, TO>>(dim3(ntm * p.ntn * p.ksplit), dim3(512), lds, s, p);
  if (rc || p.ksplit == 1) return rc;
  return launch_splitk_finalize<TO>(p, s);
}

constexpr int kHaloAuto = 5;

template <typename T, typename TO>
int dispatch_conv(const ConvParams& p, hipStream_t s, snrse_ctx& cx) {
  if (p.Cout >= 64) {
    if (p.Cout % 128 != 0) return SNRSE_EINVAL;
    if constexpr (sizeof(T) == 2) {
      const bool fits = p.bytes0 < 0x7ff00000ll && p.bytes1 < 0x7ff00000ll && p.sc_bytes0 < 0x7ff00000ll &&
                        p.sc_bytes1 < 0x7ff00000ll;
      if (cx.conv_variant != 1 && fits) {
        if (cx.conv_variant != 2 && p.ksize == 3 && halo_tile64(p)) {
          cx.last_kernel = kHaloAuto;
          return launch_halo5<T, TO>(p, s, cx);
        }
        if (p.gn_scale) return SNRSE_EINVAL;
        cx.last_kernel = 2;
        if (p.Cout % 256 == 0) return launch_glds<128, 256, T, TO>(p, s, cx);
        return launch_glds<256, 128, T, TO>(p, s, cx);
      }
    }
    if (p.gn_scale) return SNRSE_EINVAL;
    cx.last_kernel = 1;
    return launch_conv<T, TO, 128, 128, 2, 2>(p, p.Cout, s, cx);
  }
  if constexpr (sizeof(T) == 2 && sizeof(TO) == 4) {
    const bool small = cx.head_small == 2 && (long long)p.B * p.H * p.W <= 16384;
    if (cx.conv_variant != 1 && head_ok(p) && !small) {
      const bool part = cx.head_part != 0 && p.Cout == 4;
      cx.last_kernel = part ? 15 : 10;
      return launch_head(p, s, part, std::is_same_v<T, f16_t>);
    }
    if (cx.conv_variant != 1 && cx.head_small && head_small_ok(p)) {
      cx.last_kernel = 14;
      cx.last_ksplit = 1;
      return launch_head_small(p, s, false, std::is_same_v<T, f16_t>);
    }
  }
  if (p.gn_scale) return SNRSE_EINVAL;
  if (p.Cout > 16) return SNRSE_EINVAL;
  cx.last_kernel = 1;
  return launch_conv<T, TO, 128, 16, 4, 1>(p, 16, s, cx);
}

inline long long x3h_tile_count(const ConvParams& p, int tw) {
  return (long long)p.B * (p.H / (256 / tw)) * ((p.W + tw - 1) / tw) * (p.Cout / 128);
}

int dispatch_x3(const ConvParams& q, hipStream_t stream, snrse_ctx& cx, bool x3h_all) {
  if (x3h_all) {
    cx.last_kernel = 4;
    cx.last_ksplit = 1;
    ConvParams r = q;
    r.epi_nt = cx.x3_nt && stream_output(cx, (long long)q.M * q.out_ld * 4ll) != 0;
    cx.last_epi_nt = r.epi_nt;
    const int tw = (cx.x3_tw != 64 && q.H % 8 == 0 && q.W % 32 == 0) ? 32 : 64;
    cx.last_tw = tw;
    return launch_x3h(r, stream, (int)x3h_tile_count(q, tw), cx.x3_spread, tw, cx.h5_specialise != 0);
  }
  if (q.Cout <= 16 && cx.conv_variant != 1 && head_ok(q, true)) {
    cx.last_kernel = 11;
    cx.last_ksplit = 1;
    return launch_head_x3(q, stream);
  }
  if (q.Cout <= 16 && cx.conv_variant != 1 && cx.head_small && head_small_ok(q)) {
    cx.last_kernel = 14;
    cx.last_ksplit = 1;
    return launch_head_small(q, stream, true);
  }
  if (q.gn_scale) return SNRSE_EINVAL;
  cx.last_kernel = 3;
  if (q.Cout <= 16) return launch_x3<128, 16, 4, 1>(q, stream, cx);
  if (cx.x3_tile == 2) return launch_x3<256, 128, 4, 2>(q, stream, cx);
  if (cx.x3_tile == 3 && q.Cout % 256 == 0) return launch_x3<128, 256, 2, 4>(q, stream, cx);
  return launch_x3<128, 128, 2, 2>(q, stream, cx);
}

ConvParams image_range(const ConvParams& p, int b0, int nb, long long esz, long long osz) {
  ConvParams q = p;
  const long long HW = (long long)p.H * p.W, px0 = (long long)b0 * HW;
  auto off = [&](const void* ptr, long long elems, long long bytes_per) -> const void* {
    return ptr ? (const void*)((const char*)ptr + elems * bytes_per) : nullptr;
  };
  const int Cin = p.C0 + p.C1;
  q.src0 = off(p.src0, px0 * p.C0, esz);
  q.src1 = off(p.src1, px0 * p.C1, esz);
  q.sc_src = off(p.sc_src, px0 * p.Csc, esz);
  q.sc_src1 = off(p.sc_src1, px0 * p.Csc1, esz);
  q.res = off(p.res, px0 * p.res_ld, osz);
  q.comb_src = (const float*)off(p.comb_src, px0 * 4, 4);
  q.out = (void*)off(p.out, px0 * p.out_ld, osz);
  q.temb = (const float*)off(p.temb, (long long)b0 * p.temb_stride, 4);
  q.stats = p.stats ? p.stats + (size_t)b0 * SNRSE_STAT_SLOTS * p.Cout * 2 : nullptr;
  q.gn_scale = (const float*)off(p.gn_scale, (long long)b0 * Cin, 4);
  q.gn_shift = (const float*)off(p.gn_shift, (long long)b0 * Cin, 4);
  q.B = nb;
  q.M = nb * p.H * p.W;
  const long long qpix = (long long)nb * HW;
  q.bytes0 = qpix * p.C0 * esz; q.bytes1 = qpix * p.C1 * esz;
  q.sc_bytes0 = qpix * p.Csc * esz; q.sc_bytes1 = qpix * p.Csc1 * esz;
  return q;
}

}

extern "C" int snrse_conv2d(snrse_ctx* ctx, const void* src0, int C0, const void* src1, int C1, int B, int H, int W,
                            int ksize, const void* wgt, const void* sc_src, int Csc, const void* sc_src1,
                            int Csc1, const void* sc_wgt,
                            const float* bias, const float* temb, int temb_stride, const void* res,
                            int res_ld, float out_scale, const float* comb_src, const float* comb_w,
                            const float* comb_b, void* out, int Cout, int out_ld, double* stats,
                            const float* gn_scale, const float* gn_shift, int gn_act, int dtype,
                            int out_f32, hipStream_t stream) {
  snrse_ctx& cx = *snrse_ctx_resolve(ctx);
  const bool x3 = dtype == SNRSE_F32X3;
  if (x3) {
    if (Cout > 16 && Cout % 128) return SNRSE_EINVAL;
    dtype = SNRSE_F32;
    out_f32 = 0;
  }
  const long long esz = snrse_is16(dtype) ? 2 : 4, osz = (snrse_is16(dtype) && !out_f32) ? 2 : 4;
  const int KT = esz == 2 ? ConvTraits<bf16_t>::KT : ConvTraits<float>::KT;
  if (!src0 || !wgt || !out || (ksize != 1 && ksize != 3)) return SNRSE_EINVAL;
  if (C0 % KT || C1 % KT || (sc_src && (Csc % KT || Csc1 % KT))) return SNRSE_EINVAL;
  if (sc_src && Csc1 > 0 && !sc_src1) return SNRSE_EINVAL;
  if (C1 > 0 && !src1) return SNRSE_EINVAL;
  ConvParams p{};
  p.src0 = src0; p.C0 = C0; p.src1 = src1; p.C1 = C1;
  p.B = B; p.H = H; p.W = W; p.ksize = ksize; p.wgt = wgt;
  p.sc_src = sc_src; p.Csc = sc_src ? Csc : 0; p.sc_wgt = sc_wgt;
  p.sc_src1 = sc_src1; p.Csc1 = sc_src ? Csc1 : 0;
  p.bias = bias; p.temb = temb; p.temb_stride = temb_stride;
  p.res = res; p.res_ld = res_ld; p.out_scale = out_scale;
#ifdef SNRSE_STAMPS
  p.stamps = g_stamp_buf;
#else
  p.stamps = nullptr;
#endif
  p.comb_src = comb_src; p.comb_w = comb_w; p.comb_b = comb_b;
  p.out = out; p.Cout = Cout; p.out_ld = out_ld; p.M = B * H * W;
  p.stats = stats;
  p.epi_nt = 0;
  p.ws = nullptr; p.ksplit = 1;
  p.gn_scale = gn_scale; p.gn_shift = gn_shift; p.gn_act = gn_act;
  if ((gn_scale == nullptr) != (gn_shift == nullptr)) return SNRSE_EINVAL;
  const long long pix = (long long)B * H * W;
  p.bytes0 = pix * C0 * esz; p.bytes1 = pix * C1 * esz;
  p.sc_bytes0 = pix * p.Csc * esz; p.sc_bytes1 = pix * p.Csc1 * esz;
  const int npad = Cout >= 64 ? Cout : 16;
  p.wbytes = (long long)npad * ksize * ksize * (C0 + C1) * esz;
  p.sc_wbytes = (long long)npad * (p.Csc + p.Csc1) * esz;
  p.ntn = 1;
  if (p.M <= 0) return 0;
  if (stats && !cx.stats_zeroed) SNRSE_RET(hipMemsetAsync(stats, 0, sizeof(double) * 2 * SNRSE_STAT_SLOTS * (size_t)B * Cout, stream));
  if (!snrse_is16(dtype) && dtype != SNRSE_F32) return SNRSE_EINVAL;
  const bool x3h_all = x3 && ksize == 3 && H % x3h::TH == 0 && Cout % 128 == 0 &&
                       ((cx.x3_tile == 0 && x3h_tile_count(p, x3h::TW) >= 256) || cx.x3_tile == 4);
  auto run = [&](const ConvParams& q) {
    if (x3) return dispatch_x3(q, stream, cx, x3h_all);
    if (dtype == SNRSE_F16)
      return out_f32 ? dispatch_conv<f16_t, float>(q, stream, cx) : dispatch_conv<f16_t, f16_t>(q, stream, cx);
    if (dtype == SNRSE_BF16)
      return out_f32 ? dispatch_conv<bf16_t, float>(q, stream, cx) : dispatch_conv<bf16_t, bf16_t>(q, stream, cx);
    return dispatch_conv<float, float>(q, stream, cx);
  };
  const long long per_img = (long long)H * W * std::max(std::max(C0, C1), std::max(p.Csc, p.Csc1)) * esz;
  constexpr long long kLim = 0x7ff00000ll;
  cx.last_chunks = 1;
  SNRSE_RET((hipError_t)snrse_ctx_probe_mark(cx, stream, false));
  struct ProbeEnd {
    snrse_ctx& c;
    hipStream_t s;
    ~ProbeEnd() { (void)snrse_ctx_probe_mark(c, s, true); }
  } probe_end{cx, stream};
  if (per_img * B < kLim || per_img >= kLim) return run(p);
  const int chunk = (int)((kLim - 1) / per_img);
  cx.last_chunks = (B + chunk - 1) / chunk;
  for (int b0 = 0; b0 < B; b0 += chunk) {
    const int rc = run(image_range(p, b0, std::min(chunk, B - b0), esz, osz));
    if (rc) return rc;
  }
  return 0;
}

#ifdef SNRSE_STAMPS
extern "C" int snrse_debug_set_stamps(void* buf) {
  g_stamp_buf = (unsigned long long*)buf;
  return 0;
}
#endif
```

snr-aligned_diffse_amd/snrse/_lib.py:

```python
from __future__ import annotations

import ctypes as C
import os

import torch

from .build import LIB

F32, BF16, F16, F64, F32X3 = 0, 1, 2, 3, 4

_vp, _i, _f, _u64, _ll, _d = C.c_void_p, C.c_int, C.c_float, C.c_uint64, C.c_longlong, C.c_double

SIGNATURES = {
    "snrse_upfirdn2d": [_vp, _vp, _vp] + [_i] * 15 + [_vp],
    "snrse_conv2d": [_vp, _vp, _i, _vp, _i, _i, _i, _i, _i, _vp, _vp, _i, _vp, _i, _vp, _vp, _vp, _i, _vp, _i, _f,
                     _vp, _vp, _vp, _vp, _i, _i, _vp, _vp, _vp, _i, _i, _i, _vp],
    "snrse_gn_scale_shift": [_vp, _i, _vp, _i, _i, _i, _vp, _vp, _i, _f, _vp, _vp, _vp],
    "snrse_gn_stats": [_vp, _vp, _i, _vp, _i, _i, _i, _vp, _vp, _i, _vp],
    "snrse_gn_apply": [_vp, _i, _vp, _i, _i, _i, _i, _vp, _vp, _vp, _vp, _i, _f, _i, _i, _vp, _i, _vp],
    "snrse_set_option": [C.c_char_p, _i],
    "snrse_get_option": [C.c_char_p, _vp],
    "snrse_attention": [_vp, _vp, _i, _i, _i, _i, _vp],
    "snrse_temb_mlp": [_vp, _vp, _vp, _vp, _vp, _vp, _vp, _i, _i, _vp],
    "snrse_temb_dense": [_vp, _vp, _vp, _vp, _i, _i, _i, _vp],
    "snrse_temb_gfp_dense": [_vp, _vp, _vp, _vp, _vp, _i, _i, _vp],
    "snrse_input_pack": [_vp, _vp, _i, _i, _i, _vp, _vp, _i, _vp],
    "snrse_score_update": [_vp, _i, _vp, _vp, _vp, _i, _i, _i, _vp, _vp, _vp, _u64, _u64, _vp, _vp, _vp, _vp, _vp],
    "snrse_sde_update": [_vp, _vp, _vp, _vp, _u64, _u64, _vp, _i, _i, _vp, _vp, _vp],
    "snrse_axpby_noise": [_vp, _vp, _vp, _u64, _u64, _vp, _i, _i, _vp, _vp],
    "snrse_score_update_rs": [_vp, _i, _vp, _vp, _vp, _i, _i, _i, _vp, _vp, _vp, _vp, _u64, _vp, _vp, _vp, _vp, _vp],
    "snrse_sde_update_rs": [_vp, _vp, _vp, _vp, _vp, _u64, _vp, _i, _i, _vp, _vp, _vp],
    "snrse_axpby_noise_rs": [_vp, _vp, _vp, _vp, _u64, _vp, _i, _i, _vp, _vp],
    "snrse_stft_ragged": [_vp, _vp, _i, _i, _vp, _f, _i, _i, _vp, _vp],
    "snrse_absmax_ragged": [_vp, _vp, _i, _i, _vp, _vp],
    "snrse_energy_ratios_ragged": [_vp, _vp, _vp, _vp, _i, _i, _vp, _vp],
    "snrse_stft": [_vp, _i, _i, _vp, _f, _i, _i, _vp, _vp],
    "snrse_absmax": [_vp, _i, _i, _vp, _vp],
    "snrse_range_stats": [_vp, _i, _ll, _i, _vp, _vp, _i, _vp],
    "snrse_resample_poly": [_vp, _vp, _i, _ll, _i, _i, _i, _vp, _vp, _ll, _vp],
    "snrse_window_gather": [_vp, _vp, _i, _ll, _vp, _i, _i, _vp, _vp],
    "snrse_window_merge": [_vp, _i, _i, _vp, _vp, _vp, _vp, _i, _vp, _i, _vp, _ll, _vp],
    "snrse_energy_ratios": [_vp, _vp, _vp, _i, _i, _vp, _vp],
    "snrse_estoi": [_vp, _vp, _vp, _i, _ll, _vp, C.c_size_t, _vp, _vp, _vp],
    "snrse_input_conv": [_vp, _vp, _vp, _i, _i, _i, _vp, _vp, _vp, _vp, _vp, _i, _vp],
    "snrse_input_conv_x3": [_vp, _vp, _vp, _i, _i, _i, _vp, _vp, _vp, _vp, _vp, _vp],
    "snrse_spec_transform": [_vp, _vp, C.c_longlong, _i, _vp],
    "snrse_snrnet": [_vp, _i, _i] + [_vp] * 17 + [_vp, _vp, _vp],
    "snrse_istft": [_vp, _i, _i, _i, _i, _vp, _vp, _vp, _vp],
    "snrse_gn_resample": [_vp, _vp, _i, _i, _i, _i, _vp, _vp, _i, _i, _vp, _vp, _i, _vp],
    "snrse_gn_act": [_vp, _i, _vp, _i, _i, _i, _vp, _vp, _i, _vp, _i, _vp],
    "snrse_set_workspace": [_vp, C.c_size_t],
    "snrse_ctx_set_workspace": [_vp, _vp, C.c_size_t],
    "snrse_ctx_set_option": [_vp, C.c_char_p, _i],
    "snrse_ctx_get_option": [_vp, C.c_char_p, _vp],
    "snrse_ctx_probe_begin": [_vp, _i],
    "snrse_ctx_probe_read": [_vp, _vp, _vp, _i, _vp],
    "snrse_conv_wgrad": [_vp, _i, _vp, _i, _vp, _i, _i, _i, _i, _i, _vp, _vp],
    "snrse_conv_wgrad_x3": [_vp, _i, _vp, _i, _vp, _i, _i, _i, _i, _i, _vp, _vp],
    "snrse_chan_sum": [_vp, _i, _i, _i, _vp, _vp, _f, _vp],
    "snrse_gn_moments": [_vp, _i, _vp, _i, _i, _i, _i, _f, _vp, _vp, _vp],
    "snrse_gn_backward": [_vp, _i, _vp, _i, _vp, _i, _i, _i, _vp, _vp, _vp, _vp, _i, _vp, _vp, _vp, _vp, _vp, _vp],
    "snrse_bgemm": [_vp, _ll, _ll, _ll, _vp, _ll, _ll, _ll, _vp, _ll, _ll, _ll, _vp, _i, _i, _i, _i, _f, _f, _vp],
    "snrse_softmax_rows": [_vp, _vp, _ll, _i, _f, _vp],
    "snrse_softmax_bwd_rows": [_vp, _vp, _vp, _ll, _i, _f, _vp],
    "snrse_silu": [_vp, _vp, _ll, _vp],
    "snrse_silu_bwd": [_vp, _vp, _vp, _ll, _i, _vp],
    "snrse_axpby": [_vp, _vp, _ll, _f, _f, _vp],
    "snrse_scale_rows": [_vp, _vp, _vp, _i, _ll, _i, _vp],
    "snrse_gfp": [_vp, _vp, _i, _i, _vp, _vp],
    "snrse_ct_perturb": [_vp, _vp, _vp, _vp, _vp, _i, _i, _i, _vp, _vp, _vp],
    "snrse_ct_loss": [_vp, _vp, _vp, _vp, _vp, _i, _i, _i, _vp, _vp, _vp, _vp],
    "snrse_adam_ema": [_vp, _vp, _vp, _i, _f, _f, _f, _f, _f, _f, _f, _vp],
    "snrse_grad_sumsq": [_vp, _vp, _vp, _i, _vp, _vp],
    "snrse_grad_clip_coef": [_vp, _i, _f, _f, _vp, _vp],
    "snrse_adam_ema_scaled": [_vp, _vp, _vp, _i, _f, _f, _f, _f, _f, _f, _f, _vp, _vp],
    "snrse_grad_pack": [_vp, _vp, _vp, _i, _vp, _f, _vp, _vp],
    "snrse_snr_perturb": [_vp, _vp, _vp, _i, _ll, _vp, _vp],
    "snrse_snrnet_train_fwd": [_vp, _i, _i] + [_vp] * 17 + [_vp, _vp, _vp],
    "snrse_snrnet_backward": [_vp, _i, _i, _vp, _vp] + [_vp] * 8 + [_vp] + [_vp] * 17 + [_vp],
    "snrse_rk45_combine": [_vp, _vp, _vp, _vp, _i, _i, _i, _ll, _vp, _vp, _vp],
    "snrse_rk45_rownorm": [_vp, _vp, _i, _i, _vp, _vp, _vp, _d, _d, _i, _i, _ll, _vp, _vp, _vp],
    "snrse_rk45_accept": [_vp, _vp, _vp, _ll, _vp, _vp, _ll, _i, _vp],
    "snrse_active_window_sums": [_vp, _vp, _vp, _i, _ll, _i, _vp, _vp, _vp, _vp],
    "snrse_active_finalize": [_vp, _vp, _vp, _vp, _i, _ll, _i, _vp, _vp, _vp],
    "snrse_snr_mix": [_vp, _vp, _vp, _i, _ll, _vp, _i, _vp, _vp, _vp, _vp],
    "snrse_scale_to_pcm16": [_vp, _vp, _vp, _vp, _i, _ll, _vp, _vp, _vp, _vp, _vp, _vp, _vp, _vp, _vp],
}
HOUSEKEEPING = {"snrse_abi_version": ([], _i), "snrse_build_id": ([], C.c_char_p), "snrse_error_string": ([_i], C.c_char_p),
                "snrse_device_name": ([C.c_char_p, _i], _i), "snrse_snrnet_workspace": ([_i, _i], C.c_size_t),
                "snrse_snrnet_train_workspace": ([_i, _i], C.c_size_t),
                "snrse_rk45_rownorm_blocks": ([_i, _ll], _i), "snrse_resample_poly_block": ([], _i),
                "snrse_estoi_workspace": ([_i, _ll], C.c_size_t), "snrse_estoi_block": ([], _i),
                "snrse_active_windows_per_block": ([], _i),
                "snrse_ctx_create": ([], _vp), "snrse_ctx_destroy": ([_vp], None)}

_lib = None


def load(path: str | None = None) -> C.CDLL:
    global _lib
    if _lib is not None:
        return _lib
    path = path or os.environ.get("SNRSE_LIB", LIB)
    if not os.path.exists(path):
        raise OSError(f"libsnrse_hip.so not found at {path}: run __graft_entry__.build() "
                      "(or python -m snrse.build) first; there is no CPU fallback")
    lib = C.CDLL(path)
    for name, args in SIGNATURES.items():
        fn = getattr(lib, name)
        fn.argtypes = args
        fn.restype = _i
    for name, (args, res) in HOUSEKEEPING.items():
        fn = getattr(lib, name)
        fn.argtypes = args
        fn.restype = res
    _lib = lib
    for kv in filter(None, os.environ.get("SNRSE_OPTS", "").split(",")):
        k, v = kv.split("=")
        check(lib.snrse_set_option(k.strip().encode(), int(v)), f"snrse_set_option({k})")
    return lib


def exported_symbols():
    return list(SIGNATURES) + list(HOUSEKEEPING)


def check(rc: int, what: str):
    if rc != 0:
        msg = load().snrse_error_string(rc)
        raise RuntimeError(f"{what} failed: {msg.decode() if msg else rc} (code {rc})")


def call(name: str, *args):
    lib = load()
    n = len(SIGNATURES[name])
    if len(args) != n:
        raise TypeError(f"{name} takes {n} arguments, {len(args)} given")
    check(getattr(lib, name)(*args), name)
```

snr-aligned_diffse_amd/snrse/ncsnpp.py:

```python
from __future__ import annotations

import math
from dataclasses import dataclass, field

import torch

from . import ops

INV_SQRT2 = 1.0 / math.sqrt(2.0)
_NO_FUSED_INPUT = False


@dataclass
class Mod:
    kind: str
    idx: int
    cin: int = 0
    cout: int = 0
    up: bool = False
    down: bool = False
    extra: dict = field(default_factory=dict)


def build_plan(nf=128, ch_mult=(1, 1, 2, 2, 2, 2, 2), num_res_blocks=2, attn_resolutions=(16,),
               image_size=256):
    mods = []

    def add(kind, **kw):
        mods.append(Mod(kind, len(mods), **kw))

    nres = len(ch_mult)
    res = [image_size // (2 ** i) for i in range(nres)]
    add("gfp", cout=2 * nf)
    add("linear", cin=2 * nf, cout=4 * nf)
    add("linear", cin=4 * nf, cout=4 * nf)
    add("conv3x3", cin=4, cout=nf)
    hs_c = [nf]
    in_ch = nf
    for lvl in range(nres):
        for _ in range(num_res_blocks):
            out_ch = nf * ch_mult[lvl]
            add("rb", cin=in_ch, cout=out_ch)
            in_ch = out_ch
            if res[lvl] in attn_resolutions:
                add("attn", cin=in_ch, cout=in_ch)
            hs_c.append(in_ch)
        if lvl != nres - 1:
            add("rb", cin=in_ch, cout=in_ch, down=True)
            add("combine", cin=4, cout=in_ch)
            hs_c.append(in_ch)
    in_ch = hs_c[-1]
    add("rb", cin=in_ch, cout=in_ch)
    add("attn", cin=in_ch, cout=in_ch)
    add("rb", cin=in_ch, cout=in_ch)
    for lvl in reversed(range(nres)):
        for _ in range(num_res_blocks + 1):
            out_ch = nf * ch_mult[lvl]
            skip = hs_c.pop()
            add("rb", cin=in_ch + skip, cout=out_ch, extra={"c0": in_ch, "c1": skip})
            in_ch = out_ch
        if res[lvl] in attn_resolutions:
            add("attn", cin=in_ch, cout=in_ch)
        add("gn", cin=in_ch, cout=in_ch)
        add("conv3x3", cin=in_ch, cout=4)
        if lvl != 0:
            add("rb", cin=in_ch, cout=in_ch, up=True)
    assert not hs_c
    return mods


SHIPPED = dict(nf=128, ch_mult=(1, 1, 2, 2, 2, 2, 2), num_res_blocks=2, attn_resolutions=(16,), image_size=256)


def check_topology(**cfg):
    for k, v in cfg.items():
        want = SHIPPED.get(k)
        got = tuple(v) if isinstance(v, (list, tuple)) else v
        if want is not None and got != want:
            raise NotImplementedError(f"NCSNpp {k}={v!r}: the HIP executor is built for {k}={want!r} only")


def _pack3x3(w, dt, npad=None):
    co = w.shape[0]
    p = w.permute(0, 2, 3, 1).reshape(co, -1)
    if npad is not None and npad > co:
        p = torch.cat([p, p.new_zeros(npad - co, p.shape[1])], 0)
    return p.to(dt).contiguous()


def _pack1x1(w, dt, npad=None):
    return _pack3x3(w, dt, npad)


class RangeProbe:

    CAP = 512

    def __init__(self, B, device):
        self.names = {}
        self.peak = torch.zeros(self.CAP, B, device=device, dtype=torch.float32)
        self.nonfinite = torch.zeros(self.CAP, B, device=device, dtype=torch.int32)

    def add(self, name, t):
        row = self.names.setdefault(name, len(self.names))
        if row >= self.CAP:
            raise RuntimeError(f"snrse: range probe holds {self.CAP} tensors")
        ops.range_stats(t, self.peak[row], self.nonfinite[row], accumulate=True)

    def result(self):
        peak, nonfinite = self.peak.cpu(), self.nonfinite.cpu()
        return [(name, peak[row], nonfinite[row]) for name, row in self.names.items()]


class NCSNppHIP:

    def __init__(self, sd: dict, dtype=torch.float16, device="cuda", gemm="exact", **cfg):
        if not torch.cuda.is_available():
            raise RuntimeError("snrse: NCSNppHIP needs a HIP device (no CPU fallback)")
        if gemm not in ("exact", "x3") or (gemm == "x3" and dtype != torch.float32):
            raise ValueError(f"snrse: gemm={gemm!r} with dtype {dtype} (x3 is an fp32 mode)")
        self.dtype = dtype
        self.gemm = gemm
        self.device = torch.device(device)
        self._src = (sd, cfg)
        self._fallbacks = {}
        self._probe = None
        self._arena = None
        self._arenas = {}
        self.mid_hook = None
        check_topology(**cfg)
        self.plan = build_plan(**cfg)
        dev, dt = self.device, dtype
        f32 = lambda k: sd[k].detach().to(dev, torch.float32).contiguous()
        self.W = {}
        W = self.W
        W["gfp"] = f32("all_modules.0.W")
        W["l1w"], W["l1b"] = f32("all_modules.1.weight"), f32("all_modules.1.bias")
        W["l2w"], W["l2b"] = f32("all_modules.2.weight"), f32("all_modules.2.bias")
        w_in = sd["all_modules.3.weight"].detach().to(dev, torch.float32)
        col = w_in.permute(0, 2, 3, 1).reshape(w_in.shape[0], 36)
        W["in_w"] = torch.cat([col, col.new_zeros(col.shape[0], 28)], 1).to(dt).contiguous()
        W["in_b"] = f32("all_modules.3.bias")
        W["out_w"] = f32("output_layer.weight").reshape(2, 4).contiguous()
        W["out_b"] = f32("output_layer.bias")
        dense_w, dense_b, off = [], [], 0
        self.mw = {}
        for m in self.plan:
            pre = f"all_modules.{m.idx}"
            e = {}
            if m.kind == "rb":
                e["gn0_g"], e["gn0_b"] = f32(pre + ".GroupNorm_0.weight"), f32(pre + ".GroupNorm_0.bias")
                e["gn1_g"], e["gn1_b"] = f32(pre + ".GroupNorm_1.weight"), f32(pre + ".GroupNorm_1.bias")
                e["w0"] = _pack3x3(sd[pre + ".Conv_0.weight"].detach().to(dev), dt)
                e["b0"] = f32(pre + ".Conv_0.bias")
                e["w1"] = _pack3x3(sd[pre + ".Conv_1.weight"].detach().to(dev), dt)
                b1 = f32(pre + ".Conv_1.bias")
                if m.cin != m.cout or m.up or m.down:
                    e["w2"] = _pack1x1(sd[pre + ".Conv_2.weight"].detach().to(dev), dt)
                    b1 = b1 + f32(pre + ".Conv_2.bias")
                e["b1"] = b1.contiguous()
                dense_w.append(f32(pre + ".Dense_0.weight"))
                dense_b.append(f32(pre + ".Dense_0.bias"))
                e["temb_off"] = off
                off += m.cout
            elif m.kind == "attn":
                e["gn_g"], e["gn_b"] = f32(pre + ".GroupNorm_0.weight"), f32(pre + ".GroupNorm_0.bias")
                Ws = [sd[f"{pre}.NIN_{i}.W"].detach().to(dev, torch.float32) for i in range(4)]
                e["wqkv"] = torch.cat([Ws[0].t(), Ws[1].t(), Ws[2].t()], 0).to(dt).contiguous()
                e["bqkv"] = torch.cat([f32(f"{pre}.NIN_{i}.b") for i in range(3)]).contiguous()
                e["w3"] = Ws[3].t().to(dt).contiguous()
                e["b3"] = f32(pre + ".NIN_3.b")
            elif m.kind == "combine":
                e["w"] = f32(pre + ".Conv_0.weight").reshape(m.cout, 4).contiguous()
                e["b"] = f32(pre + ".Conv_0.bias")
            elif m.kind == "gn":
                e["g"], e["b"] = f32(pre + ".weight"), f32(pre + ".bias")
            elif m.kind == "conv3x3" and m.idx != 3:
                e["w"] = _pack3x3(sd[pre + ".weight"].detach().to(dev), dt, npad=16)
                e["b"] = f32(pre + ".bias")
            self.mw[m.idx] = e
        W["dense_w"] = torch.cat(dense_w, 0).contiguous()
        W["dense_b"] = torch.cat(dense_b, 0).contiguous()
        if gemm == "x3":
            W["in_w"] = ops.split_weight(W["in_w"])
            for m in self.plan:
                e = self.mw[m.idx]
                if m.kind == "rb":
                    for k in ("w0", "w1", "w2"):
                        if k in e:
                            e[k] = ops.split_weight(e[k])
                elif m.kind == "conv3x3" and "w" in e:
                    e["w"] = ops.split_weight(e["w"])
                elif m.kind == "attn":
                    e["wqkv"] = ops.split_weight(e["wqkv"])
                    e["w3"] = ops.split_weight(e["w3"])

    def fallback(self, dtype=torch.bfloat16, gemm="exact"):
        key = (dtype, gemm)
        if key == (self.dtype, self.gemm):
            return self
        fb = self._fallbacks.get(key)
        if fb is None:
            sd, cfg = self._src
            fb = self._fallbacks[key] = NCSNppHIP(sd, dtype=dtype, device=self.device, gemm=gemm, **cfg)
        return fb

    def _note(self, name, t):
        if self._probe is not None:
            self._probe.add(name, t)
        return t

    def range_report(self, x, y, t):
        probe = RangeProbe(x.shape[0], x.device)
        self._probe = probe
        try:
            self.pyramid(x, y, t)
        finally:
            self._probe = None
        return probe.result()

    def _conv(self, *a, **kw):
        out_stats = kw.pop("want_stats", True)
        src0 = a[0]
        st = ops.new_stats(src0.shape[0], a[3]) if out_stats else None
        out = ops.conv2d(*a, stats=st, **kw)
        return out, st

    def _resblock(self, m, x0, x1, dense, comb=None, comb_w=None, comb_b=None):
        e = self.mw[m.idx]
        note, p = self._note, f"{m.idx}.rb"
        mode = "up" if m.up else ("down" if m.down else "none")
        (t0, s0), (t1, s1) = x0, (x1 if x1 is not None else (None, None))
        B, H, W, _ = t0.shape
        xs_raw = None
        fused = ops.x3h_ok if self.gemm == "x3" else ops.halo_ok
        if mode == "none" and fused(t0, 3, m.cout):
            gn0 = ops.gn_scale_shift(s0, e["gn0_g"], e["gn0_b"], H * W, sums1=s1)
            h, hs_ = self._conv(t0, e["w0"], 3, m.cout, src1=t1, gn=gn0, bias=e["b0"], temb=dense,
                                temb_off=e["temb_off"])
        elif mode != "none" and t1 is None and ops.resample_ok(t0):
            gn0 = ops.gn_scale_shift(s0, e["gn0_g"], e["gn0_b"], H * W)
            a0, xs_raw = ops.gn_resample(t0, *gn0, act=True, mode=mode, want_raw="w2" in e)
            note(p + ".gn0", a0)
            if xs_raw is not None:
                note(p + ".fir", xs_raw)
            h, hs_ = self._conv(a0, e["w0"], 3, m.cout, bias=e["b0"], temb=dense, temb_off=e["temb_off"])
        else:
            a0 = note(p + ".gn0", ops.gn_apply(t0, t1, s0, e["gn0_g"], e["gn0_b"], act=True, mode=mode, sums1=s1))
            h, hs_ = self._conv(a0, e["w0"], 3, m.cout, bias=e["b0"], temb=dense, temb_off=e["temb_off"])
        note(p + ".conv0", h)
        Hh, Wh = h.shape[1], h.shape[2]
        if fused(h, 3, m.cout):
            src, gn1 = h, ops.gn_scale_shift(hs_, e["gn1_g"], e["gn1_b"], Hh * Wh)
        else:
            src, gn1 = note(p + ".gn1", ops.gn_apply(h, None, hs_, e["gn1_g"], e["gn1_b"], act=True)), None
        if "w2" in e:
            if mode != "none":
                xs0, xs1 = (note(p + ".fir", ops.fir(t0, mode)) if xs_raw is None else xs_raw), None
            else:
                xs0, xs1 = t0, t1
            out = self._conv(src, e["w1"], 3, m.cout, gn=gn1, bias=e["b1"], sc=xs0, sc1=xs1, sc_wgt=e["w2"],
                             out_scale=INV_SQRT2, comb=comb, comb_w=comb_w, comb_b=comb_b)
        else:
            assert t1 is None
            out = self._conv(src, e["w1"], 3, m.cout, gn=gn1, bias=e["b1"], res=t0, out_scale=INV_SQRT2,
                             comb=comb, comb_w=comb_w, comb_b=comb_b)
        note(p + ".conv1", out[0])
        return out

    def _attn(self, m, x):
        e = self.mw[m.idx]
        t, s = x
        note, p = self._note, f"{m.idx}.attn"
        a = note(p + ".gn", ops.gn_apply(t, None, s, e["gn_g"], e["gn_b"], act=False))
        qkv, _ = self._conv(a, e["wqkv"], 1, 3 * m.cout, bias=e["bqkv"], want_stats=False)
        o = note(p + ".out", ops.attention(note(p + ".qkv", qkv), m.cout, split=self.gemm == "x3"))
        out = self._conv(o, e["w3"], 1, m.cout, bias=e["b3"], res=t, out_scale=INV_SQRT2)
        note(p + ".nin3", out[0])
        return out

    def _pyramid_head(self, gn_m, conv_m, h, pyr_up):
        g = self.mw[gn_m.idx]
        c = self.mw[conv_m.idx]
        t, s = h
        if ops.head_ok(t, split=self.gemm == "x3"):
            gn = ops.gn_scale_shift(s, g["g"], g["b"], t.shape[1] * t.shape[2])
            return self._note(f"{conv_m.idx}.head",
                              ops.conv2d(t, c["w"], 3, 4, bias=c["b"], res=pyr_up, out_f32=True, gn=gn))
        a = self._note(f"{gn_m.idx}.gn", ops.gn_apply(t, None, s, g["g"], g["b"], act=True))
        return self._note(f"{conv_m.idx}.head", ops.conv2d(a, c["w"], 3, 4, bias=c["b"], res=pyr_up, out_f32=True))

    def temb(self, t):
        W = self.W
        temb = ops.temb_mlp(t, W["gfp"], W["l1w"], W["l1b"], W["l2w"], W["l2b"])
        return ops.temb_dense(temb, W["dense_w"], W["dense_b"])

    def pyramid(self, x, y, t):
        key = torch.cuda.current_stream(x.device).cuda_stream
        arena = self._arenas.get(key)
        if arena is None:
            arena = self._arenas[key] = ops.StatsArena(x.device)
        self._arena = arena
        with arena:
            return self._pyramid(x, y, t)

    def _pyramid(self, x, y, t):
        W = self.W
        dense = self.temb(t)
        if self.dtype in ops.H16 and ops.input_conv_ok(x) and not _NO_FUSED_INPUT:
            ht, hst, pyr_in = ops.input_conv(x, y, W["in_w"], W["in_b"])
            h = (ht, hst)
        elif self.gemm == "x3" and ops.input_conv_x3_ok(x) and not _NO_FUSED_INPUT:
            ht, hst, pyr_in = ops.input_conv_x3(x, y, W["in_w"], W["in_b"])
            h = (ht, hst)
        else:
            col, pyr_in = ops.input_pack(x, y, self.dtype)
            h = self._conv(col, W["in_w"], 1, 128, bias=W["in_b"])
        self._note("3.conv", h[0])
        hs = [h]
        plan = self.plan
        i = 4
        nres = 7
        for lvl in range(nres):
            for _ in range(2):
                h = self._resblock(plan[i], hs[-1], None, dense)
                i += 1
                if plan[i].kind == "attn":
                    h = self._attn(plan[i], h)
                    i += 1
                hs.append(h)
            if lvl != nres - 1:
                rb, cmb = plan[i], plan[i + 1]
                pyr_in = self._note(f"{cmb.idx}.combine.fir", ops.fir(pyr_in, "down"))
                ce = self.mw[cmb.idx]
                h = self._resblock(rb, hs[-1], None, dense, comb=pyr_in, comb_w=ce["w"], comb_b=ce["b"])
                i += 2
                hs.append(h)
        h = hs[-1]
        h = self._resblock(plan[i], h, None, dense); i += 1
        h = self._attn(plan[i], h); i += 1
        h = self._resblock(plan[i], h, None, dense); i += 1
        if self.mid_hook is not None:
            hook, self.mid_hook = self.mid_hook, None
            hook()
        pyr = None
        for lvl in reversed(range(nres)):
            for _ in range(3):
                h = self._resblock(plan[i], h, hs.pop(), dense)
                i += 1
            if plan[i].kind == "attn":
                h = self._attn(plan[i], h)
                i += 1
            pyr_up = None if pyr is None else self._note(f"{plan[i + 1].idx}.head.fir", ops.fir(pyr, "up"))
            pyr = self._pyramid_head(plan[i], plan[i + 1], h, pyr_up)
            i += 2
            if lvl != 0:
                h = self._resblock(plan[i], h, None, dense)
                i += 1
        assert i == len(plan) and not hs
        return pyr

    def score(self, x, y, t, score_mode=0):
        pyr = self.pyramid(x, y, t)
        _, _, sc = ops.score_update(pyr, self.W["out_w"], self.W["out_b"], t, score_mode, x, y, want_score=True)
        return sc

    def dnn(self, x, y, t):
        return -self.score(x, y, t, score_mode=0)
```

snr-aligned_diffse_amd/snrse/ops.py:

```python
from __future__ import annotations

import ctypes as C
import itertools
import math
import os
import threading
import weakref

import numpy as np
import torch

from . import _lib

F32, BF16, F16 = _lib.F32, _lib.BF16, _lib.F16
INV_SQRT2 = 1.0 / math.sqrt(2.0)
H16 = (torch.float16, torch.bfloat16)


def conv_code(act_dtype: torch.dtype, wgt_dtype: torch.dtype) -> int:
    if act_dtype == torch.float32 and wgt_dtype == torch.bfloat16:
        return _lib.F32X3
    if wgt_dtype != act_dtype:
        raise TypeError(f"snrse: conv weights {wgt_dtype} for {act_dtype} activations")
    return code(act_dtype)


def split_weight(w: torch.Tensor) -> torch.Tensor:
    n, k = w.shape
    if k % 32:
        raise ValueError(f"snrse: split weights need K % 32 == 0, got {k}")
    w = w.float().reshape(n, k // 32, 1, 32)
    hi = w.to(torch.bfloat16)
    lo = (w - hi.float()).to(torch.bfloat16)
    return torch.cat([hi, lo], 2).reshape(n, 2 * k).contiguous()


def code(dtype: torch.dtype) -> int:
    if dtype == torch.float32:
        return F32
    if dtype == torch.float16:
        return F16
    if dtype == torch.bfloat16:
        return BF16
    raise TypeError(f"snrse: unsupported dtype {dtype}")


def _ptr(t):
    return None if t is None else t.data_ptr()


def _stream():
    return torch.cuda.current_stream().cuda_stream


def current_device():
    return torch.device("cuda", torch.cuda.current_device())


def _ws_alloc(dev):
    mb = int(os.environ.get("SNRSE_WORKSPACE_MB", "128"))
    return (torch.empty(mb << 18, dtype=torch.float32, device=dev) if mb > 0 else None), mb


_CONTEXTS = weakref.WeakSet()
_CTX_SEQ = itertools.count()
_TLS = threading.local()


class LaunchContext:

    def __init__(self, device):
        lib = _lib.load()
        self.device = torch.device(device)
        self.ptr = lib.snrse_ctx_create()
        if not self.ptr:
            raise MemoryError("snrse_ctx_create failed")
        self._lib = lib
        self.ws, mb = _ws_alloc(self.device)
        _lib.call("snrse_ctx_set_workspace", self.ptr, None if self.ws is None else self.ws.data_ptr(),
                  0 if self.ws is None else mb << 20)
        self.zeroed = int(bool(self.get_option("stats_zeroed")))
        self.seq = next(_CTX_SEQ)
        _CONTEXTS.add(self)

    def set_option(self, name, value):
        _lib.call("snrse_ctx_set_option", self.ptr, name.encode(), int(value))
        if name == "stats_zeroed":
            self.zeroed = int(bool(value))

    def get_option(self, name):
        v = C.c_int(0)
        _lib.call("snrse_ctx_get_option", self.ptr, name.encode(), C.addressof(v))
        return v.value

    def __del__(self):
        try:
            self._lib.snrse_ctx_destroy(self.ptr)
        except Exception:
            pass


def _tls_contexts(dev):
    d = getattr(_TLS, "ctx", None)
    if d is None:
        d = _TLS.ctx = {}
        _TLS.lane = {}
    return d.setdefault(torch.device(dev), {})


def context(dev=None, lane=None):
    dev = current_device() if dev is None else torch.device(dev)
    ctxs = _tls_contexts(dev)
    if lane is None:
        lane = _TLS.lane.get(dev, 0)
    c = ctxs.get(lane)
    if c is None:
        c = ctxs[lane] = LaunchContext(dev)
    return c


def _cx(dev):
    return context(dev).ptr


def use_workspace_lane(lane, dev):
    dev = torch.device(dev)
    _tls_contexts(dev)
    _TLS.lane[dev] = lane
    context(dev, lane)


def _dev(*ts):
    for t in ts:
        if t is not None and not t.is_cuda:
            raise RuntimeError("snrse: HIP device tensor required (no CPU fallback)")
        if t is not None and not t.is_contiguous():
            raise RuntimeError("snrse: contiguous tensor required")


def conv2d(src0, wgt, ksize, cout, bias=None, src1=None, sc=None, sc1=None, sc_wgt=None, temb=None,
           temb_off=0, res=None, out_scale=1.0, comb=None, comb_w=None, comb_b=None, out=None,
           out_f32=False, stats=None, gn=None, gn_act=True):
    _dev(src0, src1, wgt, sc, sc1, sc_wgt, bias, res, comb, comb_w, comb_b, temb)
    cx = context(src0.device)
    B, H, W, C0 = src0.shape
    C1 = 0 if src1 is None else src1.shape[3]
    Csc = 0 if sc is None else sc.shape[3]
    Csc1 = 0 if sc1 is None else sc1.shape[3]
    odt = torch.float32 if out_f32 else src0.dtype
    if sc_wgt is not None and sc_wgt.dtype != wgt.dtype:
        raise TypeError("snrse: conv2d wgt and sc_wgt must share one layout (both split or neither)")
    if out is None:
        out = torch.empty(B, H, W, cout, device=src0.device, dtype=odt)
    _stats_zeroed(cx, stats)
    _lib.call("snrse_conv2d", cx.ptr, _ptr(src0), C0, _ptr(src1), C1, B, H, W, ksize, _ptr(wgt), _ptr(sc), Csc,
              _ptr(sc1), Csc1, _ptr(sc_wgt), _ptr(bias), None if temb is None else temb.data_ptr() + 4 * temb_off,
              0 if temb is None else temb.shape[1], _ptr(res), 0 if res is None else res.shape[-1], float(out_scale), _ptr(comb),
              _ptr(comb_w), _ptr(comb_b), out.data_ptr(), cout, out.shape[-1], _ptr(stats),
              None if gn is None else gn[0].data_ptr(), None if gn is None else gn[1].data_ptr(), int(bool(gn_act)),
              conv_code(src0.dtype, wgt.dtype), int(out_f32), _stream())
    return out


def _opt(x, name):
    return context(x.device).get_option(name)


def get_option(name):
    return context().get_option(name)


def _probe_contexts(dev, all_threads):
    own = context(dev)
    if not all_threads:
        return [own]
    others = sorted((c for c in list(_CONTEXTS) if c is not own and c.device == own.device), key=lambda c: c.seq)
    return [own] + others


def probe_begin(capacity, dev=None, all_threads=False):
    for cx in _probe_contexts(dev, all_threads):
        _lib.call("snrse_ctx_probe_begin", cx.ptr, int(capacity))


def probe_read(max_calls, dev=None, all_threads=False):
    out_ms, out_k = [], []
    for cx in _probe_contexts(dev, all_threads):
        ms = (C.c_float * max_calls)()
        kern = (C.c_int * max_calls)()
        n = C.c_int(0)
        _lib.call("snrse_ctx_probe_read", cx.ptr, C.addressof(ms), C.addressof(kern), int(max_calls),
                  C.addressof(n))
        out_ms += list(ms[:n.value])
        out_k += list(kern[:n.value])
    return out_ms, out_k


KERNELS = {1: "conv_mfma_kernel", 2: "conv_glds_kernel", 3: "conv_x3_kernel", 4: "conv_x3h_kernel",
           5: "conv_halo5_kernel",
           10: "conv_head_kernel", 11: "conv_head_x3_kernel", 14: "conv_head_small_kernel",
           15: "conv_head_part_kernel"}


def kernel_name(gen):
    return KERNELS.get(gen, f"conv_kernel_{gen}")


def conv_kernel_name():
    return kernel_name(get_option("halo_kernel"))


def halo_ok(x, ksize, cout):
    B, H, W, C = x.shape
    return (x.dtype in H16 and ksize == 3 and cout % 128 == 0 and H % 4 == 0 and W % 64 == 0
            and _opt(x, "conv_variant") in (0, 5))


def x3h_ok(x, ksize, cout):
    B, H, W, C = x.shape
    if x.dtype != torch.float32 or ksize != 3 or cout % 128 or H % 4:
        return False
    t = _opt(x, "x3_tile")
    return t == 4 or (t == 0 and B * (H // 4) * (-(-W // 64)) * (cout // 128) >= 256)


def head_ok(x, split=False):
    B, H, W, C = x.shape
    if _opt(x, "conv_variant") == 1:
        return False
    h16 = x.dtype in H16
    dt_ok = h16 or (split and x.dtype == torch.float32)
    if dt_ok and H % 8 == 0 and W % 32 == 0 and C % (64 if h16 else 32) == 0 and (not h16 or C <= 1024):
        return True
    return dt_ok and C % 256 == 0 and _opt(x, "head_small") != 0


def gn_scale_shift(sums0, gamma, beta, HW, sums1=None, groups=None, eps=1e-6):
    _dev(sums0, sums1, gamma, beta)
    B, C0 = sums0.shape[0], sums0.shape[2]
    C1 = 0 if sums1 is None else sums1.shape[2]
    C = C0 + C1
    g = groups if groups is not None else min(C // 4, 32)
    ss = torch.empty(2, B, C, device=sums0.device, dtype=torch.float32)
    scale, shift = ss[0], ss[1]
    _lib.call("snrse_gn_scale_shift", sums0.data_ptr(), C0, _ptr(sums1), C1, B, HW, gamma.data_ptr(), beta.data_ptr(),
              g, float(eps), scale.data_ptr(), shift.data_ptr(), _stream())
    return scale, shift


STAT_SLOTS = 16


def _arena_stack():
    st = getattr(_TLS, "arenas", None)
    if st is None:
        st = _TLS.arenas = []
    return st


class StatsArena:

    ALIGN = 32

    def __init__(self, device):
        self.device = torch.device(device)
        self.buf, self.off, self.need = None, 0, 0

    def __enter__(self):
        if self.buf is not None:
            self.buf.zero_()
        self.off, self.need = 0, 0
        _arena_stack().append(self)
        return self

    def __exit__(self, *exc):
        _arena_stack().remove(self)
        if self.buf is None or self.need > self.buf.numel():
            self.buf = torch.empty(self.need, dtype=torch.float64, device=self.device)
        return False

    def take(self, n):
        na = (n + self.ALIGN - 1) // self.ALIGN * self.ALIGN
        self.need += na
        if self.buf is None or self.off + na > self.buf.numel():
            return None
        t = self.buf[self.off:self.off + n]
        self.off += na
        return t


def _stats_zeroed(cx, *bufs):
    bufs = [b for b in bufs if b is not None]
    if not bufs:
        return
    z = int(all(getattr(b, "_snrse_zeroed", False) for b in bufs))
    if cx.zeroed != z:
        cx.set_option("stats_zeroed", z)


def new_stats(x_or_shape, C=None):
    if C is None:
        B, C, dev = x_or_shape.shape[0], x_or_shape.shape[-1], x_or_shape.device
    else:
        B, dev = x_or_shape, current_device()
    st = _arena_stack()
    if st and st[-1].device == torch.device(dev):
        t = st[-1].take(B * STAT_SLOTS * C * 2)
        if t is not None:
            t = t.view(B, STAT_SLOTS, C, 2)
            t._snrse_zeroed = True
            return t
    return torch.empty(B, STAT_SLOTS, C, 2, device=dev, dtype=torch.float64)


def fold_stats(st):
    return st.sum(1)


def gn_stats(src0, src1=None):
    _dev(src0, src1)
    B, H, W, C0 = src0.shape
    C1 = 0 if src1 is None else src1.shape[3]
    s0 = new_stats(src0)
    s1 = None if src1 is None else new_stats(src1)
    cx = context(src0.device)
    _stats_zeroed(cx, s0, s1)
    _lib.call("snrse_gn_stats", cx.ptr, _ptr(src0), C0, _ptr(src1), C1, B, H * W, s0.data_ptr(), _ptr(s1),
              code(src0.dtype), _stream())
    return s0, s1


MODES = {"none": 0, "down": 1, "up": 2}
GN_FUSED_MAX_HW = 512


def gn_apply(src0, src1=None, sums=None, gamma=None, beta=None, act=True, mode="none", groups=None, eps=1e-6,
             sums1=None):
    if isinstance(sums, tuple):
        sums, sums1 = sums
    _dev(src0, src1, sums, sums1, gamma, beta)
    B, H, W, C0 = src0.shape
    C1 = 0 if src1 is None else src1.shape[3]
    C = C0 + C1
    m = MODES[mode]
    small = m == 0 and H * W <= GN_FUSED_MAX_HW
    if sums is not None and (m == 0 or resample_ok(src0)) and not small:
        scale, shift = gn_scale_shift(sums, gamma, beta, H * W, sums1=sums1, groups=groups, eps=eps)
        if m == 0:
            return gn_act(src0, src1, scale, shift, act=act)
        if src1 is None and resample_ok(src0):
            return gn_resample(src0, scale, shift, act=act, mode=mode)[0]
    Ho, Wo = (H // 2, W // 2) if m == 1 else ((2 * H, 2 * W) if m == 2 else (H, W))
    out = torch.empty(B, Ho, Wo, C, device=src0.device, dtype=src0.dtype)
    g = groups if groups is not None else min(C // 4, 32)
    _lib.call("snrse_gn_apply", _ptr(src0), C0, _ptr(src1), C1, B, H, W, _ptr(sums), _ptr(sums1), _ptr(gamma),
              _ptr(beta), g, float(eps), int(bool(act)), m, out.data_ptr(), code(src0.dtype), _stream())
    return out


def resample_ok(x):
    C = x.shape[3]
    if x.dtype in H16:
        return C % 16 == 0
    return x.dtype == torch.float32 and C % 4 == 0 and 64 % (C // 4) == 0


def gn_resample(x, scale=None, shift=None, act=True, mode="down", want_raw=False):
    _dev(x, scale, shift)
    if x.dtype not in (torch.float16, torch.bfloat16, torch.float32):
        raise TypeError("snrse: gn_resample takes fp16, bf16 or f32 activations")
    B, H, W, C = x.shape
    m = MODES[mode]
    if m == 0:
        raise ValueError("snrse: gn_resample mode must be 'down' or 'up'")
    Ho, Wo = (H // 2, W // 2) if m == 1 else (2 * H, 2 * W)
    oa = torch.empty(B, Ho, Wo, C, device=x.device, dtype=x.dtype)
    orw = torch.empty_like(oa) if want_raw else None
    _lib.call("snrse_gn_resample", _cx(x.device), x.data_ptr(), C, B, H, W, _ptr(scale), _ptr(shift), int(bool(act)), m,
              oa.data_ptr(), _ptr(orw), code(x.dtype), _stream())
    return oa, orw


def gn_act(src0, src1=None, scale=None, shift=None, act=True):
    _dev(src0, src1, scale, shift)
    B, H, W, C0 = src0.shape
    C1 = 0 if src1 is None else src1.shape[3]
    out = torch.empty(B, H, W, C0 + C1, device=src0.device, dtype=src0.dtype)
    _lib.call("snrse_gn_act", src0.data_ptr(), C0, _ptr(src1), C1, B, H * W, _ptr(scale), _ptr(shift),
              int(bool(act)), out.data_ptr(), code(src0.dtype), _stream())
    return out


def fir(x, mode):
    return gn_apply(x, act=False, mode=mode)


def attention(qkv, C=256, split=False):
    _dev(qkv)
    B, L = qkv.shape[0], qkv.shape[1] * (qkv.shape[2] if qkv.dim() == 4 else 1)
    out = torch.empty(*qkv.shape[:-1], C, device=qkv.device, dtype=qkv.dtype)
    if split and qkv.dtype != torch.float32:
        raise TypeError("snrse: split attention takes fp32 q, k, v")
    _lib.call("snrse_attention", qkv.data_ptr(), out.data_ptr(), B, L, C, _lib.F32X3 if split else code(qkv.dtype),
              _stream())
    return out


def temb_mlp(t, Wg, W1, b1, W2, b2, fused=False):
    _dev(t, Wg, W1, b1, W2, b2)
    B = t.shape[0]
    out = torch.empty(B, W2.shape[0], device=t.device, dtype=torch.float32)
    if fused:
        _lib.call("snrse_temb_mlp", t.data_ptr(), Wg.data_ptr(), W1.data_ptr(), b1.data_ptr(), W2.data_ptr(),
                  b2.data_ptr(), out.data_ptr(), B, Wg.shape[0], _stream())
        return out
    a = torch.empty(B, W1.shape[0], device=t.device, dtype=torch.float32)
    _lib.call("snrse_temb_gfp_dense", t.data_ptr(), Wg.data_ptr(), W1.data_ptr(), b1.data_ptr(), a.data_ptr(), B,
              Wg.shape[0], _stream())
    _lib.call("snrse_temb_dense", a.data_ptr(), W2.data_ptr(), b2.data_ptr(), out.data_ptr(), B, W2.shape[0],
              W2.shape[1], _stream())
    return out


def temb_dense(temb, W, bias):
    _dev(temb, W, bias)
    B, D = temb.shape
    R = W.shape[0]
    out = torch.empty(B, R, device=temb.device, dtype=torch.float32)
    _lib.call("snrse_temb_dense", temb.data_ptr(), W.data_ptr(), bias.data_ptr(), out.data_ptr(), B, R, D,
              _stream())
    return out


def input_conv_ok(x):
    B, F, T = x.shape[0], x.shape[-2], x.shape[-1]
    return T % 64 == 0 and (F * T // 64) % 16 == 0


def input_conv(x, y, wgt, bias):
    _dev(x, y, wgt, bias)
    if wgt.dtype not in H16:
        raise TypeError(f"snrse: input_conv takes fp16 / bf16 weights, got {wgt.dtype}")
    B, F, T = x.shape[0], x.shape[-2], x.shape[-1]
    h = torch.empty(B, F, T, 128, device=x.device, dtype=wgt.dtype)
    pyr = torch.empty(B, F, T, 4, device=x.device, dtype=torch.float32)
    st = new_stats(B, 128)
    cx = context(x.device)
    _stats_zeroed(cx, st)
    _lib.call("snrse_input_conv", cx.ptr, x.data_ptr(), y.data_ptr(), B, F, T, wgt.data_ptr(), bias.data_ptr(),
              h.data_ptr(), pyr.data_ptr(), st.data_ptr(), code(wgt.dtype), _stream())
    return h, st, pyr


def input_conv_x3_ok(x):
    return input_conv_ok(x) and x.shape[-1] <= 1024


def input_conv_x3(x, y, wgt_split, bias):
    _dev(x, y, wgt_split, bias)
    B, F, T = x.shape[0], x.shape[-2], x.shape[-1]
    h = torch.empty(B, F, T, 128, device=x.device, dtype=torch.float32)
    pyr = torch.empty(B, F, T, 4, device=x.device, dtype=torch.float32)
    st = new_stats(B, 128)
    cx = context(x.device)
# ... 604 lines not shown
```

Measured before the change: 14.35 utt/s.

## Fuse GroupNorm stats and next-layer normalize+SiLU into split-K finalize

Adds a split-K finalize kernel for small-spatial fp16 convolutions. In one block per batch and channel slice it sums the K-split partials, applies the epilogue, reduces the GroupNorm statistics, and writes up to three normalized (optionally SiLU-activated) copies for the consuming layers. The model passes the next plan step so resblocks and attention can request these emitted activations. This is meant to remove the separate stats and gn_apply launches, along with their extra reads of the conv output, at low-resolution levels. The cost is more dispatch complexity, reliance on context state attached through a new API, and a fallback to the unfused path when the shape constraints are not met.

```diff
diff --git a/include/snrse.h b/include/snrse.h
--- a/include/snrse.h
+++ b/include/snrse.h
@@ -37,6 +37,14 @@
                  const float* comb_w, const float* comb_b, void* out, int Cout, int out_ld,
                  double* stats, const float* gn_scale, const float* gn_shift, int gn_act, int dtype,
                  int out_f32, hipStream_t stream);
+
+int snrse_ctx_attach_gn(snrse_ctx* ctx, const float* gamma, const float* beta, int C, int groups, float eps, int act,
+                        void* dst, int dst_ld, int dst_coff);
+
+int snrse_splitk_finalize(snrse_ctx* ctx, const float* ws, int ksplit, int B, int H, int W, int Cout, const float* bias,
+                          const float* temb, int temb_stride, const void* res, int res_ld, float out_scale,
+                          const float* comb_src, const float* comb_w, const float* comb_b, void* out, int out_ld,
+                          double* stats, int dtype, int out_f32, hipStream_t stream);
 
 #define SNRSE_STAT_SLOTS 16
 
diff --git a/snr-aligned_diffse_amd/csrc/abi.cpp b/snr-aligned_diffse_amd/csrc/abi.cpp
--- a/snr-aligned_diffse_amd/csrc/abi.cpp
+++ b/snr-aligned_diffse_amd/csrc/abi.cpp
@@ -55,6 +55,7 @@
   if (name_is(name, "head_small")) return &c.head_small;
   if (name_is(name, "head_part")) return &c.head_part;
   if (name_is(name, "gn_slice")) return &c.gn_slice;
+  if (name_is(name, "fin_gn")) return &c.fin_gn;
   return nullptr;
 }
 
@@ -77,6 +78,7 @@
   if (name_is(name, "last_epi_nt")) { *value = c.last_epi_nt; return 0; }
   if (name_is(name, "last_chunks")) { *value = c.last_chunks; return 0; }
   if (name_is(name, "last_tw")) { *value = c.last_tw; return 0; }
+  if (name_is(name, "last_fin_gn")) { *value = c.last_fin_gn; return 0; }
   return SNRSE_EINVAL;
 }
 
@@ -164,6 +166,8 @@
   c->last_epi_nt = 0;
   c->last_chunks = 1;
   c->last_tw = 0;
+  c->last_fin_gn = 0;
+  c->n_emit = 0;
   c->probe_ev = nullptr;
   c->probe_kernel = nullptr;
   c->probe_cap = c->probe_n = 0;
@@ -185,6 +189,16 @@
   return get_option(*snrse_ctx_resolve(const_cast<snrse_ctx*>(ctx)), name, value);
 }
 
+extern "C" int snrse_ctx_attach_gn(snrse_ctx* ctx, const float* gamma, const float* beta, int C, int groups, float eps,
+                                   int act, void* dst, int dst_ld, int dst_coff) {
+  snrse_ctx& c = *snrse_ctx_resolve(ctx);
+  if (!gamma || !beta || !dst || groups <= 0 || C <= 0 || C % groups || dst_coff < 0 || dst_ld <= 0 ||
+      c.n_emit >= SNRSE_MAX_EMIT)
+    return SNRSE_EINVAL;
+  c.emit[c.n_emit++] = snrse_gn_emit{gamma, beta, dst, dst_ld, dst_coff, C, C / groups, act ? 1 : 0, eps};
+  return 0;
+}
+
 extern "C" int snrse_set_workspace(void* ptr, size_t bytes) { return set_workspace(g_default_ctx, ptr, bytes); }
 extern "C" int snrse_set_option(const char* name, int value) { return set_option(g_default_ctx, name, value); }
 extern "C" int snrse_get_option(const char* name, int* value) { return get_option(g_default_ctx, name, value); }
diff --git a/snr-aligned_diffse_amd/csrc/common.h b/snr-aligned_diffse_amd/csrc/common.h
--- a/snr-aligned_diffse_amd/csrc/common.h
+++ b/snr-aligned_diffse_amd/csrc/common.h
@@ -144,6 +144,17 @@
 inline bool snrse_is16(int dtype) { return dtype == SNRSE_BF16 || dtype == SNRSE_F16; }
 
 #define SNRSE_STAT_SLOTS 16
+
+struct snrse_gn_emit {
+  const float* gamma;
+  const float* beta;
+  void* dst;
+  int dst_ld, dst_coff;
+  int C, cg;
+  int act;
+  float eps;
+};
+#define SNRSE_MAX_EMIT 3
 
 struct snrse_ctx {
   int conv_variant = 0;
@@ -165,9 +176,12 @@
   int head_part = 1;
   int gn_slice = 1;
   int ic_lds = 3;
+  int fin_gn = 1;
   float* ws = nullptr;
   size_t ws_bytes = 0;
-  int last_kernel = 0, last_ksplit = 1, last_epi_nt = 0, last_chunks = 1, last_tw = 0;
+  int n_emit = 0;
+  snrse_gn_emit emit[SNRSE_MAX_EMIT] = {};
+  int last_kernel = 0, last_ksplit = 1, last_epi_nt = 0, last_chunks = 1, last_tw = 0, last_fin_gn = 0;
   hipEvent_t* probe_ev = nullptr;
   int* probe_kernel = nullptr;
   int probe_cap = 0, probe_n = 0;
diff --git a/snr-aligned_diffse_amd/csrc/conv.hip b/snr-aligned_diffse_amd/csrc/conv.hip
--- a/snr-aligned_diffse_amd/csrc/conv.hip
+++ b/snr-aligned_diffse_amd/csrc/conv.hip
@@ -1220,6 +1220,95 @@
                            (float*)(smem + 8 * (64 * 68 * 4)), wm, b_lo == b_hi ? b_lo : -1, n0);
 }
 
+SNRSE_DEV void splitk_terms(const ConvParams& p, int b, int n, float (&add)[8], float (&cw)[8][4], float (&cb)[8]) {
+#pragma unroll
+  for (int k = 0; k < 8; ++k) {
+    add[k] = (p.bias ? p.bias[n + k] : 0.f) + (p.temb ? p.temb[(size_t)b * p.temb_stride + n + k] : 0.f);
+    cb[k] = 0.f;
+    cw[k][0] = cw[k][1] = cw[k][2] = cw[k][3] = 0.f;
+    if (p.comb_src) {
+      cw[k][0] = p.comb_w[(n + k) * 4 + 0];
+      cw[k][1] = p.comb_w[(n + k) * 4 + 1];
+      cw[k][2] = p.comb_w[(n + k) * 4 + 2];
+      cw[k][3] = p.comb_w[(n + k) * 4 + 3];
+      cb[k] = p.comb_b[n + k];
+    }
+  }
+}
+
+template <int PPT, int N>
+SNRSE_DEV void splitk_add(const float* const (&w)[PPT], size_t plane, int s, f32x4 (&a0)[PPT], f32x4 (&a1)[PPT]) {
+  f32x4 q[PPT][N][2];
+#pragma unroll
+  for (int i = 0; i < PPT; ++i)
+#pragma unroll
+    for (int u = 0; u < N; ++u) {
+      q[i][u][0] = *(const f32x4*)(w[i] + (s + u) * plane);
+      q[i][u][1] = *(const f32x4*)(w[i] + (s + u) * plane + 4);
+    }
+#pragma unroll
+  for (int i = 0; i < PPT; ++i)
+#pragma unroll
+    for (int u = 0; u < N; ++u) {
+      a0[i] += q[i][u][0];
+      a1[i] += q[i][u][1];
+    }
+}
+
+template <int PPT>
+SNRSE_DEV void splitk_sum(const ConvParams& p, const float* const (&w)[PPT], f32x4 (&a0)[PPT], f32x4 (&a1)[PPT]) {
+  constexpr int NB = PPT >= 8 ? 2 : (PPT >= 4 ? 4 : 8);
+  const size_t plane = (size_t)p.M * p.Cout;
+#pragma unroll
+  for (int i = 0; i < PPT; ++i) {
+    a0[i] = *(const f32x4*)w[i];
+    a1[i] = *(const f32x4*)(w[i] + 4);
+  }
+  int s = 1;
+  for (; s + NB <= p.ksplit; s += NB) splitk_add<PPT, NB>(w, plane, s, a0, a1);
+  switch (p.ksplit - s) {
+#define SNRSE_SPLITK_REST(N) \
+  case (N):                  \
+    if constexpr (NB > (N)) splitk_add<PPT, (N)>(w, plane, s, a0, a1); \
+    break;
+    SNRSE_SPLITK_REST(7)
+    SNRSE_SPLITK_REST(6)
+    SNRSE_SPLITK_REST(5)
+    SNRSE_SPLITK_REST(4)
+    SNRSE_SPLITK_REST(3)
+    SNRSE_SPLITK_REST(2)
+    SNRSE_SPLITK_REST(1)
+#undef SNRSE_SPLITK_REST
+    default: break;
+  }
+}
+
+template <typename TO>
+SNRSE_DEV void splitk_epilogue(const ConvParams& p, size_t m, int n, const f32x4 a0, const f32x4 a1,
+                               const float (&add)[8], const float (&cw)[8][4], const float (&cb)[8], float (&v)[8]) {
+#pragma unroll
+  for (int k = 0; k < 4; ++k) {
+    v[k] = a0[k] + add[k];
+    v[4 + k] = a1[k] + add[4 + k];
+  }
+  if (p.res) {
+    if constexpr (sizeof(TO) == 2) {
+      epi_residual<TO>(*(const u32x4*)((const TO*)p.res + m * p.res_ld + n), v);
+    } else {
+      const float* rp = (const float*)p.res + m * p.res_ld + n;
+#pragma unroll
+      for (int k = 0; k < 8; ++k) v[k] += rp[k];
+    }
+  }
+#pragma unroll
+  for (int k = 0; k < 8; ++k) v[k] *= p.out_scale;
+  if (p.comb_src) {
+    const f32x4 q = *(const f32x4*)(p.comb_src + m * 4);
+#pragma unroll
+    for (int k = 0; k < 8; ++k) v[k] += q[0] * cw[k][0] + q[1] * cw[k][1] + q[2] * cw[k][2] + q[3] * cw[k][3] + cb[k];
+  }
+}
+
 template <typename TO>
 __global__ __launch_bounds__(256) void conv_splitk_finalize(ConvParams p, int ppb) {
   __shared__ float red[16 * 256];
@@ -1230,20 +1319,11 @@
   const int cl = (threadIdx.x & 15) * 8, r0 = threadIdx.x >> 4;
   const int n = blockIdx.y * 128 + cl;
   float add[8], cw[8][4], cb[8], s1[8], s2[8];
+  splitk_terms(p, b, n, add, cw, cb);
 #pragma unroll
   for (int k = 0; k < 8; ++k) {
-    add[k] = (p.bias ? p.bias[n + k] : 0.f) + (p.temb ? p.temb[(size_t)b * p.temb_stride + n + k] : 0.f);
     s1[k] = 0.f;
     s2[k] = 0.f;
-    cb[k] = 0.f;
-    cw[k][0] = cw[k][1] = cw[k][2] = cw[k][3] = 0.f;
-    if (p.comb_src) {
-      cw[k][0] = p.comb_w[(n + k) * 4 + 0];
-      cw[k][1] = p.comb_w[(n + k) * 4 + 1];
-      cw[k][2] = p.comb_w[(n + k) * 4 + 2];
-      cw[k][3] = p.comb_w[(n + k) * 4 + 3];
-      cb[k] = p.comb_b[n + k];
-    }
   }
   const size_t plane = (size_t)p.M * p.Cout;
   for (int px = px0 + r0; px < px1; px += 16) {
@@ -1269,27 +1349,7 @@
       a1 += *(const f32x4*)(w + s * plane + 4);
     }
     float v[8];
-#pragma unroll
-    for (int k = 0; k < 4; ++k) {
-      v[k] = a0[k] + add[k];
-      v[4 + k] = a1[k] + add[4 + k];
-    }
-    if (p.res) {
-      if constexpr (sizeof(TO) == 2) {
-        epi_residual<TO>(*(const u32x4*)((const TO*)p.res + m * p.res_ld + n), v);
-      } else {
-        const float* rp = (const float*)p.res + m * p.res_ld + n;
-#pragma unroll
-        for (int k = 0; k < 8; ++k) v[k] += rp[k];
-      }
-    }
-#pragma unroll
-    for (int k = 0; k < 8; ++k) v[k] *= p.out_scale;
-    if (p.comb_src) {
-      const f32x4 q = *(const f32x4*)(p.comb_src + m * 4);
-#pragma unroll
-      for (int k = 0; k < 8; ++k) v[k] += q[0] * cw[k][0] + q[1] * cw[k][1] + q[2] * cw[k][2] + q[3] * cw[k][3] + cb[k];
-    }
+    splitk_epilogue<TO>(p, m, n, a0, a1, add, cw, cb, v);
     if constexpr (sizeof(TO) == 2) {
       *(u32x4*)((TO*)p.out + m * p.out_ld + n) = epi_pack<TO>(v);
     } else {
@@ -1317,6 +1377,131 @@
     unsafeAtomicAdd(&p.stats[stat_idx(b, blockIdx.x & (SNRSE_STAT_SLOTS - 1), blockIdx.y * 128 + (t >> 1), p.Cout) +
                              (t & 1)],
                     (double)a);
+  }
+}
+
+struct FinGnEmits {
+  int n;
+  snrse_gn_emit e[SNRSE_MAX_EMIT];
+};
+
+template <typename TO, int CS, int PPT>
+__global__ __launch_bounds__(512) void conv_splitk_finalize_gn(ConvParams p, FinGnEmits g) {
+  static_assert(sizeof(TO) == 2 && CS % 8 == 0 && 64 % (CS / 8) == 0, "16-bit output, 8-channel lanes");
+  constexpr int LPP = CS / 8, ROWS = 512 / LPP;
+  __shared__ double wred[8][CS][2];
+  __shared__ double chs[CS][2];
+  __shared__ float aff[SNRSE_MAX_EMIT][2][CS];
+  const int HW = p.H * p.W;
+  const int b = blockIdx.x, c0 = blockIdx.y * CS, t = threadIdx.x;
+  const int cl = (t % LPP) * 8, r0 = t / LPP;
+  const int n = c0 + cl;
+  float add[8], cw[8][4], cb[8], s1[8], s2[8];
+  splitk_terms(p, b, n, add, cw, cb);
+#pragma unroll
+  for (int k = 0; k < 8; ++k) {
+    s1[k] = 0.f;
+    s2[k] = 0.f;
+  }
+  u32x4 keep[PPT];
+  if ((t & ~63) / LPP < HW) {
+    const float* w[PPT];
+    f32x4 a0[PPT], a1[PPT];
+#pragma unroll
+    for (int i = 0; i < PPT; ++i) w[i] = p.ws + ((size_t)b * HW + min(r0 + i * ROWS, HW - 1)) * p.Cout + n;
+    splitk_sum<PPT>(p, w, a0, a1);
+#pragma unroll
+    for (int i = 0; i < PPT; ++i) {
+      const int px = r0 + i * ROWS;
+      const bool ok = px < HW;
+      const size_t m = (size_t)b * HW + (ok ? px : HW - 1);
+      float v[8];
+      splitk_epilogue<TO>(p, m, n, a0[i], a1[i], add, cw, cb, v);
+      keep[i] = epi_pack<TO>(v);
+      if (ok) {
+        if (p.out) *(u32x4*)((TO*)p.out + m * p.out_ld + n) = keep[i];
+#pragma unroll
+        for (int k = 0; k < 8; ++k) {
+          s1[k] += v[k];
+          s2[k] = fmaf(v[k], v[k], s2[k]);
+        }
+      }
+    }
+  }
+  if (!p.stats && g.n == 0) return;
+  double d1[8], d2[8];
+#pragma unroll
+  for (int k = 0; k < 8; ++k) {
+    d1[k] = (double)s1[k];
+    d2[k] = (double)s2[k];
+  }
+#pragma unroll
+  for (int o = LPP; o < 64; o <<= 1) {
+#pragma unroll
+    for (int k = 0; k < 8; ++k) {
+      d1[k] += __shfl_xor(d1[k], o, 64);
+      d2[k] += __shfl_xor(d2[k], o, 64);
+    }
+  }
+  if ((t & 63) < LPP) {
+#pragma unroll
+    for (int k = 0; k < 8; ++k) {
+      wred[t >> 6][cl + k][0] = d1[k];
+      wred[t >> 6][cl + k][1] = d2[k];
+    }
+  }
+  __syncthreads();
+  if (t < 2 * CS) {
+    double a = 0.0;
+#pragma unroll
+    for (int w = 0; w < 8; ++w) a += wred[w][t >> 1][t & 1];
+    chs[t >> 1][t & 1] = a;
+    if (p.stats) p.stats[stat_idx(b, 0, c0 + (t >> 1), p.Cout) + (t & 1)] = a;
+  }
+  if (g.n == 0) return;
+  __syncthreads();
+  for (int i = t; i < g.n * CS; i += 512) {
+    const int j = i / CS, c = i - j * CS;
+    const snrse_gn_emit& e = g.e[j];
+    const int k0 = c / e.cg * e.cg;
+    double s = 0.0, ss = 0.0;
+    for (int k = k0; k < k0 + e.cg; ++k) {
+      s += chs[k][0];
+      ss += chs[k][1];
+    }
+    const double cnt = (double)e.cg * HW;
+    const double mean = s / cnt;
+    double var = ss / cnt - mean * mean;
+    if (var < 0.0) var = 0.0;
+    const float rstd = (float)(1.0 / sqrt(var + (double)e.eps));
+    const float scl = rstd * e.gamma[e.dst_coff + c0 + c];
+    aff[j][0][c] = scl;
+    aff[j][1][c] = e.beta[e.dst_coff + c0 + c] - (float)mean * scl;
+  }
+  __syncthreads();
+  for (int j = 0; j < g.n; ++j) {
+    const snrse_gn_emit& e = g.e[j];
+    float sc[8], sh[8];
+#pragma unroll
+    for (int k = 0; k < 8; ++k) {
+      sc[k] = aff[j][0][cl + k];
+      sh[k] = aff[j][1][cl + k];
+    }
+    TO* const dst = (TO*)e.dst + e.dst_coff + n;
+#pragma unroll
+    for (int i = 0; i < PPT; ++i) {
+      const int px = r0 + i * ROWS;
+      if (px < HW) {
+        float x[8];
+        unpack8<TO>(keep[i], x);
+#pragma unroll
+        for (int k = 0; k < 8; ++k) {
+          const float y = fmaf(x[k], sc[k], sh[k]);
+          x[k] = e.act ? silu(y) : y;
+        }
+        *(u32x4*)(dst + ((size_t)b * HW + px) * e.dst_ld) = pack8<TO>(x);
+      }
+    }
   }
 }
 
@@ -1741,6 +1926,52 @@
   hipLaunchKernelGGL((conv_splitk_finalize<TO>), dim3(p.B * ((HW + ppb - 1) / ppb), p.Cout / 128), dim3(256), 0, s, p,
                      ppb);
   return (int)hipGetLastError();
+}
+
+int fin_gn_slice(const ConvParams& p, size_t osz, const snrse_ctx& cx) {
+  if (!cx.fin_gn || p.ksplit <= 1 || osz != 2 || p.H * p.W > 512 || p.Cout % 64) return 0;
+  int cgmax = 1;
+  for (int i = 0; i < cx.n_emit; ++i) {
+    const snrse_gn_emit& e = cx.emit[i];
+    if (e.cg > 64 || 64 % e.cg || e.dst_coff % e.cg || e.dst_coff % 8 || e.dst_ld % 8 || e.dst_coff + p.Cout > e.dst_ld ||
+        e.dst_coff + p.Cout > e.C)
+      return 0;
+    cgmax = std::max(cgmax, e.cg);
+  }
+  return (cx.fin_gn != 2 && p.B * (p.Cout / 64) < 256 && cgmax <= 32) ? 32 : 64;
+}
+
+template <typename TO, int CS>
+int launch_splitk_finalize_gn_cs(const ConvParams& p, const FinGnEmits& g, hipStream_t s) {
+  constexpr int ROWS = 512 / (CS / 8);
+  const int need = (p.H * p.W + ROWS - 1) / ROWS;
+  const dim3 grid(p.B, p.Cout / CS);
+#define SNRSE_FIN_GN(PPT)                                                                          \
+  if (need <= (PPT)) {                                                                             \
+    hipLaunchKernelGGL((conv_splitk_finalize_gn<TO, CS, (PPT)>), grid, dim3(512), 0, s, p, g);     \
+    return (int)hipGetLastError();                                                                 \
+  }
+  SNRSE_FIN_GN(1)
+  SNRSE_FIN_GN(2)
+  SNRSE_FIN_GN(4)
+  if constexpr (ROWS < 128) {
+    SNRSE_FIN_GN(8)
+  }
+#undef SNRSE_FIN_GN
+  return SNRSE_EINVAL;
+}
+
+template <typename TO>
+int launch_splitk_finalize_gn(const ConvParams& p, int cs, snrse_ctx& cx, hipStream_t s) {
+  if constexpr (sizeof(TO) == 2) {
+    FinGnEmits g{};
+    g.n = cx.n_emit;
+    for (int i = 0; i < cx.n_emit; ++i) g.e[i] = cx.emit[i];
+    cx.last_fin_gn = 1;
+    return cs == 32 ? launch_splitk_finalize_gn_cs<TO, 32>(p, g, s) : launch_splitk_finalize_gn_cs<TO, 64>(p, g, s);
+  } else {
+    return SNRSE_EINVAL;
+  }
 }
 
 inline int k_tiles(const ConvParams& p, int KT) {
@@ -1913,8 +2144,11 @@
   p.ksplit = choose_ksplit(p, ntm * p.ntn, k_tiles(p, 64), cx);
   p.ws = cx.ws;
   cx.last_ksplit = p.ksplit;
+  const int cs = fin_gn_slice(p, sizeof(TO), cx);
+  if (!cs && (cx.n_emit || !p.out)) return SNRSE_EINVAL;
   const int rc = launch_dyn_lds<conv_glds_kernel<BM, BN, T, TO>>(dim3(ntm * p.ntn * p.ksplit), dim3(512), lds, s, p);
   if (rc || p.ksplit == 1) return rc;
+  if (cs) return launch_splitk_finalize_gn<TO>(p, cs, cx, s);
   return launch_splitk_finalize<TO>(p, s);
 }
 
@@ -1922,6 +2156,7 @@
 
 template <typename T, typename TO>
 int dispatch_conv(const ConvParams& p, hipStream_t s, snrse_ctx& cx) {
+  const bool att = cx.n_emit || !p.out;
   if (p.Cout >= 64) {
     if (p.Cout % 128 != 0) return SNRSE_EINVAL;
     if constexpr (sizeof(T) == 2) {
@@ -1929,6 +2164,7 @@
                         p.sc_bytes1 < 0x7ff00000ll;
       if (cx.conv_variant != 1 && fits) {
         if (cx.conv_variant != 2 && p.ksize == 3 && halo_tile64(p)) {
+          if (att) return SNRSE_EINVAL;
           cx.last_kernel = kHaloAuto;
           return launch_halo5<T, TO>(p, s, cx);
         }
@@ -1938,10 +2174,11 @@
         return launch_glds<256, 128, T, TO>(p, s, cx);
       }
     }
-    if (p.gn_scale) return SNRSE_EINVAL;
+    if (p.gn_scale || att) return SNRSE_EINVAL;
     cx.last_kernel = 1;
     return launch_conv<T, TO, 128, 128, 2, 2>(p, p.Cout, s, cx);
   }
+  if (att) return SNRSE_EINVAL;
   if constexpr (sizeof(T) == 2 && sizeof(TO) == 4) {
     const bool small = cx.head_small == 2 && (long long)p.B * p.H * p.W <= 16384;
     if (cx.conv_variant != 1 && head_ok(p) && !small) {
@@ -1966,6 +2203,7 @@
 }
 
 int dispatch_x3(const ConvParams& q, hipStream_t stream, snrse_ctx& cx, bool x3h_all) {
+  if (cx.n_emit || !q.out) return SNRSE_EINVAL;
   if (x3h_all) {
     cx.last_kernel = 4;
     cx.last_ksplit = 1;
@@ -2031,6 +2269,11 @@
                             const float* gn_scale, const float* gn_shift, int gn_act, int dtype,
                             int out_f32, hipStream_t stream) {
   snrse_ctx& cx = *snrse_ctx_resolve(ctx);
+  struct EmitEnd {
+    snrse_ctx& c;
+    ~EmitEnd() { c.n_emit = 0; }
+  } emit_end{cx};
+  cx.last_fin_gn = 0;
   const bool x3 = dtype == SNRSE_F32X3;
   if (x3) {
     if (Cout > 16 && Cout % 128) return SNRSE_EINVAL;
@@ -2039,7 +2282,7 @@
   }
   const long long esz = snrse_is16(dtype) ? 2 : 4, osz = (snrse_is16(dtype) && !out_f32) ? 2 : 4;
   const int KT = esz == 2 ? ConvTraits<bf16_t>::KT : ConvTraits<float>::KT;
-  if (!src0 || !wgt || !out || (ksize != 1 && ksize != 3)) return SNRSE_EINVAL;
+  if (!src0 || !wgt || (!out && !cx.n_emit) || (ksize != 1 && ksize != 3)) return SNRSE_EINVAL;
   if (C0 % KT || C1 % KT || (sc_src && (Csc % KT || Csc1 % KT))) return SNRSE_EINVAL;
   if (sc_src && Csc1 > 0 && !sc_src1) return SNRSE_EINVAL;
   if (C1 > 0 && !src1) return SNRSE_EINVAL;
@@ -2092,6 +2335,7 @@
     ~ProbeEnd() { (void)snrse_ctx_probe_mark(c, s, true); }
   } probe_end{cx, stream};
   if (per_img * B < kLim || per_img >= kLim) return run(p);
+  if (cx.n_emit || !out) return SNRSE_EINVAL;
   const int chunk = (int)((kLim - 1) / per_img);
   cx.last_chunks = (B + chunk - 1) / chunk;
   for (int b0 = 0; b0 < B; b0 += chunk) {
@@ -2101,6 +2345,37 @@
   return 0;
 }
 
+extern "C" int snrse_splitk_finalize(snrse_ctx* ctx, const float* ws, int ksplit, int B, int H, int W, int Cout,
+                                     const float* bias, const float* temb, int temb_stride, const void* res, int res_ld,
+                                     float out_scale, const float* comb_src, const float* comb_w, const float* comb_b,
+                                     void* out, int out_ld, double* stats, int dtype, int out_f32,
+                                     hipStream_t stream) {
+  snrse_ctx& cx = *snrse_ctx_resolve(ctx);
+  struct EmitEnd {
+    snrse_ctx& c;
+    ~EmitEnd() { c.n_emit = 0; }
+  } emit_end{cx};
+  cx.last_fin_gn = 0;
+  if (!ws || ksplit < 1 || B <= 0 || H <= 0 || W <= 0 || Cout <= 0 || Cout % 64 || out_ld < Cout) return SNRSE_EINVAL;
+  if (!snrse_is16(dtype) && dtype != SNRSE_F32) return SNRSE_EINVAL;
+  const bool o32 = out_f32 || dtype == SNRSE_F32;
+  ConvParams p{};
+  p.B = B; p.H = H; p.W = W; p.M = B * H * W; p.Cout = Cout;
+  p.bias = bias; p.temb = temb; p.temb_stride = temb_stride;
+  p.res = res; p.res_ld = res_ld; p.out_scale = out_scale;
+  p.comb_src = comb_src; p.comb_w = comb_w; p.comb_b = comb_b;
+  p.out = out; p.out_ld = out_ld; p.stats = stats;
+  p.ws = const_cast<float*>(ws); p.ksplit = ksplit;
+  if (stats && !cx.stats_zeroed)
+    SNRSE_RET(hipMemsetAsync(stats, 0, sizeof(double) * 2 * SNRSE_STAT_SLOTS * (size_t)B * Cout, stream));
+  const int cs = fin_gn_slice(p, o32 ? 4 : 2, cx);
+  if (cs) return dtype == SNRSE_F16 ? launch_splitk_finalize_gn<f16_t>(p, cs, cx, stream)
+                                    : launch_splitk_finalize_gn<bf16_t>(p, cs, cx, stream);
+  if (!out || Cout % 128) return SNRSE_EINVAL;
+  if (o32) return launch_splitk_finalize<float>(p, stream);
+  return dtype == SNRSE_F16 ? launch_splitk_finalize<f16_t>(p, stream) : launch_splitk_finalize<bf16_t>(p, stream);
+}
+
 #ifdef SNRSE_STAMPS
 extern "C" int snrse_debug_set_stamps(void* buf) {
   g_stamp_buf = (unsigned long long*)buf;
diff --git a/snr-aligned_diffse_amd/snrse/_lib.py b/snr-aligned_diffse_amd/snrse/_lib.py
--- a/snr-aligned_diffse_amd/snrse/_lib.py
+++ b/snr-aligned_diffse_amd/snrse/_lib.py
@@ -15,6 +15,9 @@
     "snrse_upfirdn2d": [_vp, _vp, _vp] + [_i] * 15 + [_vp],
     "snrse_conv2d": [_vp, _vp, _i, _vp, _i, _i, _i, _i, _i, _vp, _vp, _i, _vp, _i, _vp, _vp, _vp, _i, _vp, _i, _f,
                      _vp, _vp, _vp, _vp, _i, _i, _vp, _vp, _vp, _i, _i, _i, _vp],
+    "snrse_ctx_attach_gn": [_vp, _vp, _vp, _i, _i, _f, _i, _vp, _i, _i],
+    "snrse_splitk_finalize": [_vp, _vp, _i, _i, _i, _i, _i, _vp, _vp, _i, _vp, _i, _f, _vp, _vp, _vp, _vp, _i, _vp, _i,
+                              _i, _vp],
     "snrse_gn_scale_shift": [_vp, _i, _vp, _i, _i, _i, _vp, _vp, _i, _f, _vp, _vp, _vp],
     "snrse_gn_stats": [_vp, _vp, _i, _vp, _i, _i, _i, _vp, _vp, _i, _vp],
     "snrse_gn_apply": [_vp, _i, _vp, _i, _i, _i, _i, _vp, _vp, _vp, _vp, _i, _f, _i, _i, _vp, _i, _vp],
diff --git a/snr-aligned_diffse_amd/snrse/ncsnpp.py b/snr-aligned_diffse_amd/snrse/ncsnpp.py
--- a/snr-aligned_diffse_amd/snrse/ncsnpp.py
+++ b/snr-aligned_diffse_amd/snrse/ncsnpp.py
@@ -226,63 +226,99 @@
         out = ops.conv2d(*a, stats=st, **kw)
         return out, st
 
-    def _resblock(self, m, x0, x1, dense, comb=None, comb_w=None, comb_b=None):
+    def _gn_emit(self, nxt, like, ksize, cout, cin, csc=0):
+        if nxt is None or self.dtype not in ops.H16:
+            return None
+        e = self.mw[nxt.idx]
+        if nxt.kind == "rb" and not (nxt.up or nxt.down) and "c0" not in nxt.extra and not ops.halo_ok(like, 3, nxt.cout):
+            em = ops.GnEmit(e["gn0_g"], e["gn0_b"], act=True)
+        elif nxt.kind == "attn":
+            em = ops.GnEmit(e["gn_g"], e["gn_b"], act=False)
+        else:
+            return None
+        return em if em.C == cout and ops.fin_gn_ok(like, ksize, cout, cin, csc, [em]) else None
+
+    def _resblock(self, m, x0, x1, dense, comb=None, comb_w=None, comb_b=None, nxt=None):
         e = self.mw[m.idx]
         note, p = self._note, f"{m.idx}.rb"
         mode = "up" if m.up else ("down" if m.down else "none")
-        (t0, s0), (t1, s1) = x0, (x1 if x1 is not None else (None, None))
+        (t0, s0), (t1, s1) = x0[:2], (x1[:2] if x1 is not None else (None, None))
+        pre = x0[2] if len(x0) > 2 and x1 is None and mode == "none" else None
         B, H, W, _ = t0.shape
         xs_raw = None
         fused = ops.x3h_ok if self.gemm == "x3" else ops.halo_ok
+        a0, src1, gn0 = t0, t1, None
         if mode == "none" and fused(t0, 3, m.cout):
             gn0 = ops.gn_scale_shift(s0, e["gn0_g"], e["gn0_b"], H * W, sums1=s1)
-            h, hs_ = self._conv(t0, e["w0"], 3, m.cout, src1=t1, gn=gn0, bias=e["b0"], temb=dense,
-                                temb_off=e["temb_off"])
         elif mode != "none" and t1 is None and ops.resample_ok(t0):
-            gn0 = ops.gn_scale_shift(s0, e["gn0_g"], e["gn0_b"], H * W)
-            a0, xs_raw = ops.gn_resample(t0, *gn0, act=True, mode=mode, want_raw="w2" in e)
+            a0, xs_raw = ops.gn_resample(t0, *ops.gn_scale_shift(s0, e["gn0_g"], e["gn0_b"], H * W), act=True, mode=mode,
+                                         want_raw="w2" in e)
             note(p + ".gn0", a0)
             if xs_raw is not None:
                 note(p + ".fir", xs_raw)
-            h, hs_ = self._conv(a0, e["w0"], 3, m.cout, bias=e["b0"], temb=dense, temb_off=e["temb_off"])
         else:
-            a0 = note(p + ".gn0", ops.gn_apply(t0, t1, s0, e["gn0_g"], e["gn0_b"], act=True, mode=mode, sums1=s1))
-            h, hs_ = self._conv(a0, e["w0"], 3, m.cout, bias=e["b0"], temb=dense, temb_off=e["temb_off"])
-        note(p + ".conv0", h)
-        Hh, Wh = h.shape[1], h.shape[2]
-        if fused(h, 3, m.cout):
-            src, gn1 = h, ops.gn_scale_shift(hs_, e["gn1_g"], e["gn1_b"], Hh * Wh)
+            a0 = pre if pre is not None else ops.gn_apply(t0, t1, s0, e["gn0_g"], e["gn0_b"], act=True, mode=mode,
+                                                          sums1=s1)
+            note(p + ".gn0", a0)
+            src1 = None
+        kw0 = dict(src1=src1, gn=gn0, bias=e["b0"], temb=dense, temb_off=e["temb_off"])
+        em = None
+        if self.dtype in ops.H16 and gn0 is None and not fused(a0, 3, m.cout):
+            em = ops.GnEmit(e["gn1_g"], e["gn1_b"], act=True)
+            em = em if ops.fin_gn_ok(a0, 3, m.cout, a0.shape[3], 0, [em]) else None
+        if em is not None:
+            h, (src,) = ops.conv2d(a0, e["w0"], 3, m.cout, emit=[em], want_raw=self._probe is not None, **kw0)
+            if h is not None:
+                note(p + ".conv0", h)
+            note(p + ".gn1", src)
+            gn1 = None
         else:
-            src, gn1 = note(p + ".gn1", ops.gn_apply(h, None, hs_, e["gn1_g"], e["gn1_b"], act=True)), None
+            h, hs_ = self._conv(a0, e["w0"], 3, m.cout, **kw0)
+            note(p + ".conv0", h)
+            if fused(h, 3, m.cout):
+                src, gn1 = h, ops.gn_scale_shift(hs_, e["gn1_g"], e["gn1_b"], h.shape[1] * h.shape[2])
+            else:
+                src, gn1 = note(p + ".gn1", ops.gn_apply(h, None, hs_, e["gn1_g"], e["gn1_b"], act=True)), None
         if "w2" in e:
             if mode != "none":
                 xs0, xs1 = (note(p + ".fir", ops.fir(t0, mode)) if xs_raw is None else xs_raw), None
             else:
                 xs0, xs1 = t0, t1
-            out = self._conv(src, e["w1"], 3, m.cout, gn=gn1, bias=e["b1"], sc=xs0, sc1=xs1, sc_wgt=e["w2"],
-                             out_scale=INV_SQRT2, comb=comb, comb_w=comb_w, comb_b=comb_b)
+            csc = xs0.shape[3] + (0 if xs1 is None else xs1.shape[3])
+            kw = dict(sc=xs0, sc1=xs1, sc_wgt=e["w2"])
         else:
             assert t1 is None
-            out = self._conv(src, e["w1"], 3, m.cout, gn=gn1, bias=e["b1"], res=t0, out_scale=INV_SQRT2,
-                             comb=comb, comb_w=comb_w, comb_b=comb_b)
-        note(p + ".conv1", out[0])
-        return out
-
-    def _attn(self, m, x):
+            csc, kw = 0, dict(res=t0)
+        em = None if gn1 is not None else self._gn_emit(nxt, src, 3, m.cout, src.shape[3], csc)
+        out = self._conv(src, e["w1"], 3, m.cout, gn=gn1, bias=e["b1"], out_scale=INV_SQRT2, comb=comb, comb_w=comb_w,
+                         comb_b=comb_b, emit=None if em is None else [em], **kw)
+        return self._emitted(out, em, p + ".conv1")
+
+    def _emitted(self, out, em, name):
+        if em is None:
+            self._note(name, out[0])
+            return out[0], out[1], None
+        (t, (a,)), st = out
+        self._note(name, t)
+        return t, st, a
+
+    def _attn(self, m, x, nxt=None):
         e = self.mw[m.idx]
-        t, s = x
+        t, s = x[:2]
         note, p = self._note, f"{m.idx}.attn"
-        a = note(p + ".gn", ops.gn_apply(t, None, s, e["gn_g"], e["gn_b"], act=False))
+        a = x[2] if len(x) > 2 and x[2] is not None else ops.gn_apply(t, None, s, e["gn_g"], e["gn_b"], act=False)
+        note(p + ".gn", a)
         qkv, _ = self._conv(a, e["wqkv"], 1, 3 * m.cout, bias=e["bqkv"], want_stats=False)
         o = note(p + ".out", ops.attention(note(p + ".qkv", qkv), m.cout, split=self.gemm == "x3"))
-        out = self._conv(o, e["w3"], 1, m.cout, bias=e["b3"], res=t, out_scale=INV_SQRT2)
-        note(p + ".nin3", out[0])
-        return out
+        em = self._gn_emit(nxt, o, 1, m.cout, o.shape[3])
+        out = self._conv(o, e["w3"], 1, m.cout, bias=e["b3"], res=t, out_scale=INV_SQRT2,
+                         emit=None if em is None else [em])
+        return self._emitted(out, em, p + ".nin3")
 
     def _pyramid_head(self, gn_m, conv_m, h, pyr_up):
         g = self.mw[gn_m.idx]
         c = self.mw[conv_m.idx]
-        t, s = h
+        t, s = h[:2]
         if ops.head_ok(t, split=self.gemm == "x3"):
             gn = ops.gn_scale_shift(s, g["g"], g["b"], t.shape[1] * t.shape[2])
             return self._note(f"{conv_m.idx}.head",
@@ -323,22 +359,21 @@
         nres = 7
         for lvl in range(nres):
             for _ in range(2):
-                h = self._resblock(plan[i], hs[-1], None, dense)
+                h = self._resblock(plan[i], h, None, dense, nxt=plan[i + 1])
                 i += 1
                 if plan[i].kind == "attn":
-                    h = self._attn(plan[i], h)
+                    h = self._attn(plan[i], h, nxt=plan[i + 1])
                     i += 1
-                hs.append(h)
+                hs.append(h[:2])
             if lvl != nres - 1:
                 rb, cmb = plan[i], plan[i + 1]
                 pyr_in = self._note(f"{cmb.idx}.combine.fir", ops.fir(pyr_in, "down"))
                 ce = self.mw[cmb.idx]
-                h = self._resblock(rb, hs[-1], None, dense, comb=pyr_in, comb_w=ce["w"], comb_b=ce["b"])
+                h = self._resblock(rb, h, None, dense, comb=pyr_in, comb_w=ce["w"], comb_b=ce["b"], nxt=plan[i + 2])
                 i += 2
-                hs.append(h)
-        h = hs[-1]
-        h = self._resblock(plan[i], h, None, dense); i += 1
-        h = self._attn(plan[i], h); i += 1
+                hs.append(h[:2])
+        h = self._resblock(plan[i], h, None, dense, nxt=plan[i + 1]); i += 1
+        h = self._attn(plan[i], h, nxt=plan[i + 1]); i += 1
         h = self._resblock(plan[i], h, None, dense); i += 1
         if self.mid_hook is not None:
             hook, self.mid_hook = self.mid_hook, None
@@ -346,7 +381,7 @@
         pyr = None
         for lvl in reversed(range(nres)):
             for _ in range(3):
-                h = self._resblock(plan[i], h, hs.pop(), dense)
+                h = self._resblock(plan[i], h, hs.pop(), dense, nxt=plan[i + 1])
                 i += 1
             if plan[i].kind == "attn":
                 h = self._attn(plan[i], h)
diff --git a/snr-aligned_diffse_amd/snrse/ops.py b/snr-aligned_diffse_amd/snrse/ops.py
--- a/snr-aligned_diffse_amd/snrse/ops.py
+++ b/snr-aligned_diffse_amd/snrse/ops.py
@@ -138,9 +138,83 @@
             raise RuntimeError("snrse: contiguous tensor required")
 
 
+class GnEmit:
+
+    def __init__(self, gamma, beta, act=True, dst=None, coff=0, groups=None, eps=1e-6):
+        self.gamma, self.beta, self.act, self.dst, self.coff, self.eps = gamma, beta, bool(act), dst, int(coff), eps
+        self.C = gamma.numel()
+        self.groups = groups if groups is not None else min(self.C // 4, 32)
+        self.cg = self.C // self.groups
+
+
+FIN_GN_MAX_HW = 512
+MAX_EMIT = 3
+
+
+def glds_ksplit(x, ksize, cout, cin, csc=0, out_f32=False):
+    B, H, W, _ = x.shape
+    cx = context(x.device)
+    variant = cx.get_option("conv_variant")
+    if x.dtype not in H16 or cout < 64 or cout % 128 or variant == 1:
+        return 0
+    if B * H * W * max(cin, csc, 1) * 2 >= 0x7ff00000:
+        return 0
+    if variant != 2 and ksize == 3 and H % 4 == 0 and W % 64 == 0:
+        return 0
+    M = B * H * W
+    bm, bn = (128, 256) if cout % 256 == 0 else (256, 128)
+    tiles = -(-M // bm) * (cout // bn)
+    nk = ksize * ksize * (cin // 64) + csc // 64
+    target = cx.get_option("splitk_target")
+    if not cx.get_option("splitk") or cx.ws is None or tiles >= target * 3 // 4:
+        return 1
+    s = min(-(-target // tiles), nk // 4)
+    plane = M * cout * 4
+    if s * plane > cx.ws.numel() * 4:
+        s = cx.ws.numel() * 4 // plane
+    return s if s >= 2 else 1
+
+
+def fin_gn_ok(x, ksize, cout, cin, csc=0, emit=(), out_f32=False):
+    B, H, W, _ = x.shape
+    if out_f32 or H * W > FIN_GN_MAX_HW or cout % 64 or len(emit) > MAX_EMIT or not _opt(x, "fin_gn"):
+        return False
+    for e in emit:
+        ld = cout if e.dst is None else e.dst.shape[-1]
+        if e.C % e.groups or e.cg > 64 or 64 % e.cg or e.coff % e.cg or e.coff % 8 or ld % 8 or e.coff + cout > ld \
+                or e.coff + cout > e.C:
+            return False
+    return glds_ksplit(x, ksize, cout, cin, csc) > 1
+
+
+def _attach(cx, emit, B, H, W, cout, dtype, dev):
+    acts = []
+    for e in emit:
+        _dev(e.gamma, e.beta, e.dst)
+        dst = e.dst if e.dst is not None else torch.empty(B, H, W, cout, device=dev, dtype=dtype)
+        if dst.dtype != dtype or tuple(dst.shape[:3]) != (B, H, W):
+            raise ValueError("snrse: GnEmit dst must be [B, H, W, .] of the conv's output dtype")
+        _lib.call("snrse_ctx_attach_gn", cx.ptr, e.gamma.data_ptr(), e.beta.data_ptr(), e.C, e.groups, float(e.eps),
+                  int(e.act), dst.data_ptr(), dst.shape[-1], e.coff)
+        acts.append(dst)
+    return acts
+
+
+def _emit_unfused(out, st, e):
+    cout = out.shape[-1]
+    whole = e.coff == 0 and e.C == cout
+    g = e.gamma if whole else e.gamma[e.coff:e.coff + cout].contiguous()
+    b = e.beta if whole else e.beta[e.coff:e.coff + cout].contiguous()
+    a = gn_apply(out, None, st, g, b, act=e.act, groups=cout // e.cg, eps=e.eps)
+    if e.dst is None:
+        return a
+    e.dst[..., e.coff:e.coff + cout].copy_(a)
+    return e.dst
+
+
 def conv2d(src0, wgt, ksize, cout, bias=None, src1=None, sc=None, sc1=None, sc_wgt=None, temb=None,
            temb_off=0, res=None, out_scale=1.0, comb=None, comb_w=None, comb_b=None, out=None,
-           out_f32=False, stats=None, gn=None, gn_act=True):
+           out_f32=False, stats=None, gn=None, gn_act=True, emit=None, want_raw=True):
     _dev(src0, src1, wgt, sc, sc1, sc_wgt, bias, res, comb, comb_w, comb_b, temb)
     cx = context(src0.device)
     B, H, W, C0 = src0.shape
@@ -150,16 +224,54 @@
     odt = torch.float32 if out_f32 else src0.dtype
     if sc_wgt is not None and sc_wgt.dtype != wgt.dtype:
         raise TypeError("snrse: conv2d wgt and sc_wgt must share one layout (both split or neither)")
-    if out is None:
+    acts = None
+    if emit is not None:
+        kw = dict(bias=bias, src1=src1, sc=sc, sc1=sc1, sc_wgt=sc_wgt, temb=temb, temb_off=temb_off, res=res,
+                  out_scale=out_scale, comb=comb, comb_w=comb_w, comb_b=comb_b, out=out, out_f32=out_f32, gn=gn,
+                  gn_act=gn_act)
+        if gn is not None or not fin_gn_ok(src0, ksize, cout, C0 + C1, Csc + Csc1, emit, out_f32):
+            st = stats if stats is not None else new_stats(B, cout)
+            out = conv2d(src0, wgt, ksize, cout, stats=st, **kw)
+            return out, [_emit_unfused(out, st, e) for e in emit]
+        if not emit:
+            return conv2d(src0, wgt, ksize, cout, stats=stats, **kw), []
+        acts = _attach(cx, emit, B, H, W, cout, odt, src0.device)
+    if out is None and (want_raw or acts is None):
         out = torch.empty(B, H, W, cout, device=src0.device, dtype=odt)
     _stats_zeroed(cx, stats)
+    _conv2d_call(cx, src0, C0, src1, C1, B, H, W, ksize, wgt, sc, Csc, sc1, Csc1, sc_wgt, bias, temb, temb_off, res,
+                 out_scale, comb, comb_w, comb_b, out, cout, stats, gn, gn_act, out_f32)
+    if acts is None:
+        return out
+    if not cx.get_option("last_fin_gn"):
+        raise RuntimeError("snrse: conv2d with emit= did not take the fused finalize")
+    return out, acts
+
+
+def _conv2d_call(cx, src0, C0, src1, C1, B, H, W, ksize, wgt, sc, Csc, sc1, Csc1, sc_wgt, bias, temb, temb_off, res,
+                 out_scale, comb, comb_w, comb_b, out, cout, stats, gn, gn_act, out_f32):
     _lib.call("snrse_conv2d", cx.ptr, _ptr(src0), C0, _ptr(src1), C1, B, H, W, ksize, _ptr(wgt), _ptr(sc), Csc,
               _ptr(sc1), Csc1, _ptr(sc_wgt), _ptr(bias), None if temb is None else temb.data_ptr() + 4 * temb_off,
               0 if temb is None else temb.shape[1], _ptr(res), 0 if res is None else res.shape[-1], float(out_scale), _ptr(comb),
-              _ptr(comb_w), _ptr(comb_b), out.data_ptr(), cout, out.shape[-1], _ptr(stats),
+              _ptr(comb_w), _ptr(comb_b), _ptr(out), cout, cout if out is None else out.shape[-1], _ptr(stats),
               None if gn is None else gn[0].data_ptr(), None if gn is None else gn[1].data_ptr(), int(bool(gn_act)),
               conv_code(src0.dtype, wgt.dtype), int(out_f32), _stream())
-    return out
+
+
+def splitk_finalize(planes, dtype=torch.float16, bias=None, temb=None, temb_off=0, res=None, out_scale=1.0, comb=None,
+                    comb_w=None, comb_b=None, out_f32=False, stats=None, emit=()):
+    _dev(planes, bias, temb, res, comb, comb_w, comb_b, stats)
+    ks, B, H, W, cout = planes.shape
+    cx = context(planes.device)
+    odt = torch.float32 if out_f32 else dtype
+    out = torch.empty(B, H, W, cout, device=planes.device, dtype=odt)
+    acts = _attach(cx, emit, B, H, W, cout, odt, planes.device)
+    _stats_zeroed(cx, stats)
+    _lib.call("snrse_splitk_finalize", cx.ptr, planes.data_ptr(), ks, B, H, W, cout, _ptr(bias),
+              None if temb is None else temb.data_ptr() + 4 * temb_off, 0 if temb is None else temb.shape[1], _ptr(res),
+              0 if res is None else res.shape[-1], float(out_scale), _ptr(comb), _ptr(comb_w), _ptr(comb_b),
+              out.data_ptr(), cout, _ptr(stats), code(dtype), int(out_f32), _stream())
+    return out, acts, bool(cx.get_option("last_fin_gn"))
 
 
 def _opt(x, name):
```

After: 14.40 utt/s, median of 6. About the same (+0.3%).
